# itxtx/normalizing-flows-study

Measured on AMD Instinct MI355X. Metric: log_prob samples/sec/GPU + test-NLL match; RealNVP d=2 and MAF d=63, higher is better.
Workload: dtype fp32

## Files before the change

### include/nfx.h

```cpp
#ifndef NFX_H
#define NFX_H

#include <stddef.h>
#include <stdint.h>

#ifdef __cplusplus
extern "C" {
#endif

#define NFX_ABI_VERSION 3

#define NFX_OK 0
#define NFX_EINVAL (-1)
#define NFX_EUNSUPPORTED (-2)
#define NFX_ELAUNCH (-3)

#define NFX_FORWARD 1
#define NFX_INVERSE (-1)

#define NFX_MAF_INVERSE 0
#define NFX_IAF_FORWARD 1
#define NFX_MAF_FORWARD 2
#define NFX_IAF_INVERSE 3

typedef struct NfxMlpRaw {
    const float* w[4];
    const float* b[4];
    const float* mask[4];
    const float* bn_w[3];
    const float* bn_b[3];
    const float* bn_rm[3];
    const float* bn_rv[3];
    float bn_eps;
    int n_layers;
} NfxMlpRaw;

int nfx_abi_version(void);
const char* nfx_last_error(void);
const char* nfx_last_kernel(void);
int nfx_debug_fill_lds(uint32_t bits, void* stream);

size_t nfx_affine_packed_floats(int d, int H);
int nfx_affine_pack(const NfxMlpRaw* s_net, const NfxMlpRaw* b_net, const float* mask, int d,
                    int H, float* packed, void* stream);
int nfx_affine_coupling(const float* packed, const float* in, float* out, float* log_det,
                        int64_t B, int d, int H, int direction, int accumulate, void* stream);
int nfx_affine_coupling_logprob(const float* packed, const float* in, float* out, float* log_det,
                                float* logp, double* sums, void* workspace, int64_t B, int d,
                                int H, int accumulate, void* stream);
#define NFX_AFFINE_AUTO 0
#define NFX_AFFINE_STREAMING 1
#define NFX_AFFINE_SMALL 2
int nfx_affine_kernel_policy(int policy);

int nfx_affine_chain_supported(int64_t B, int d, int H);
int nfx_affine_chain(const float* const* packs, int n_layers, const float* in, float* out,
                     float* log_det, int64_t B, int d, int H, int direction, int accumulate,
                     void* stream);
int nfx_affine_chain_logprob(const float* const* packs, int n_layers, const float* in, float* out,
                             float* log_det, float* logp, double* sums, void* workspace, int64_t B,
                             int d, int H, int accumulate, void* stream);
int nfx_affine_chain_sample(const float* const* packs, int n_layers, uint64_t seed, uint64_t* rng_state,
                            float* z, float* x, float* log_det, int64_t B, int d, int H, void* stream);

size_t nfx_spline_packed_floats(int d, int H, int K);
int nfx_spline_pack(const NfxMlpRaw* param_net, const float* mask, int d, int H, int K,
                    float* packed, void* stream);
int nfx_spline_coupling(const float* packed, const float* in, float* out, float* log_det,
                        int64_t B, int d, int H, int K, float bound, float min_bin_width,
                        float min_bin_height, float min_derivative, int rescale,
                        float data_min, float data_max, int direction, int accumulate,
                        void* stream);
int nfx_spline_coupling_logprob(const float* packed, const float* in, float* out, float* log_det,
                                float* logp, double* sums, void* workspace, int64_t B, int d,
                                int H, int K, float bound, float min_bin_width,
                                float min_bin_height, float min_derivative, int rescale,
                                float data_min, float data_max, int accumulate, void* stream);

int nfx_spline_chain_supported(int64_t B, int d, int H, int K);
int nfx_spline_chain(const float* const* packs, int n_layers, const float* in, float* out, float* log_det,
                     int64_t B, int d, int H, int K, float bound, float min_bin_width, float min_bin_height,
                     float min_derivative, int direction, int accumulate, void* stream);
int nfx_spline_chain_logprob(const float* const* packs, int n_layers, const float* in, float* out,
                             float* log_det, float* logp, double* sums, void* workspace, int64_t B, int d,
                             int H, int K, float bound, float min_bin_width, float min_bin_height,
                             float min_derivative, int accumulate, void* stream);
int nfx_spline_chain_sample(const float* const* packs, int n_layers, uint64_t seed, uint64_t* rng_state,
                            float* z, float* x, float* log_det, int64_t B, int d, int H, int K, float bound,
                            float min_bin_width, float min_bin_height, float min_derivative, void* stream);

int nfx_rqs_unit(const float* in, const float* widths, const float* heights,
                 const float* derivatives, float* out, float* log_det, int64_t N, int K,
                 float min_bin_width, float min_bin_height, float min_derivative, int inverse,
                 void* stream);
int nfx_rqs_unit_backward(const float* in, const float* widths, const float* heights,
                          const float* derivatives, const float* grad_out, const float* grad_log_det,
                          float* grad_in, float* grad_widths, float* grad_heights, float* grad_derivatives,
                          int64_t N, int K, float min_bin_width, float min_bin_height, float min_derivative,
                          int inverse, void* stream);

size_t nfx_arqs_packed_floats(int d, int H, int K);
int nfx_arqs_pack(const NfxMlpRaw* made, int d, int H, int K, float* packed, void* stream);
int nfx_arqs(const float* packed, const float* in, float* out, float* log_det, int64_t B, int d,
             int H, int K, float min_bin_width, float min_bin_height, float min_derivative,
             int rescale, double data_min, double data_max, int direction, int accumulate,
             void* stream);

int nfx_base_normal(uint64_t seed, uint64_t* rng_state, float* z, int64_t B, int d, void* stream);

size_t nfx_made_packed_floats(int d, int H);
int nfx_made_pack(const NfxMlpRaw* net, int d, int H, float* packed, void* stream);
int nfx_made_pack_parallel(const NfxMlpRaw* net, int d, int H, float* packed, void* stream);
int nfx_made_pack_sequential(int d, int H, float* packed, void* stream);
int nfx_made_affine(const float* packed, const float* in, float* out, float* log_det,
                    int64_t B, int d, int H, int variant, int accumulate, void* stream);
#define NFX_MADE_SEQ_AUTO 0
#define NFX_MADE_SEQ_SEGMENT 1
#define NFX_MADE_SEQ_WAVE 2
#define NFX_MADE_SEQ_PUSH 3
int nfx_made_seq_policy(int policy);
int nfx_made_affine_logprob(const float* packed, const float* in, float* out, float* log_det,
                            float* logp, double* sums, void* workspace, int64_t B, int d, int H,
                            int variant, int accumulate, void* stream);
int nfx_made_sample_supported(int d, int H, int variant);
int nfx_made_affine_sample(const float* packed, uint64_t seed, uint64_t* rng_state, float* z, float* x,
                           float* log_det, int64_t B, int d, int H, void* stream);

int nfx_made_pack_backward(const NfxMlpRaw* net, int d, int H, float* packed, void* stream);
size_t nfx_made_backward_factor_floats(int64_t B, int d, int H);
int64_t nfx_made_backward_max_batch(int d, int H);
int nfx_made_affine_backward(const float* packed, const float* in, const float* grad_out,
                             const float* grad_log_det, float* grad_in, float* factors, int64_t B,
                             int d, int H, int variant, void* stream);

int nfx_made_seq_backward(const float* packed, const float* in, const float* grad_out,
                          const float* grad_log_det, float* grad_in, float* factors, int64_t B,
                          int d, int H, int variant, void* stream);
int64_t nfx_made_factor_pitch(int64_t B);
size_t nfx_made_param_floats(int d, int H);
size_t nfx_made_wgrad_workspace_bytes(int64_t B, int d, int H);
int nfx_made_backward_weights(const float* factors, int64_t B, int d, int H,
                              const float* const* masks, float* grads, void* workspace,
                              void* stream);

size_t nfx_spline_backward_packed_floats(int d, int H, int K);
size_t nfx_spline_backward_param_floats(int d, int H, int K);
size_t nfx_spline_backward_workspace_bytes(int64_t B, int d, int H, int K);
int nfx_spline_pack_backward(const NfxMlpRaw* net, const float* mask, int d, int H, int K,
                             float* packed, void* stream);
int nfx_spline_coupling_backward(const float* packed, const float* mask, const float* in,
                                 const float* grad_out, const float* grad_log_det, float* grad_in,
                                 float* grads, void* workspace, int64_t B, int d, int H, int K,
                                 int n_transformed, float bound, float min_bin_width,
                                 float min_bin_height, float min_derivative, int direction,
                                 void* stream);

size_t nfx_affine_train_pack_floats(int d, int H);
size_t nfx_affine_train_stats_doubles(int H);
size_t nfx_affine_train_grad_doubles(int d, int H);
size_t nfx_affine_train_param_floats(int d, int H);
size_t nfx_affine_train_workspace_bytes(int64_t B, int d, int H);
int nfx_affine_train_pack(const NfxMlpRaw* s_net, const NfxMlpRaw* b_net, const float* mask,
                          const double* stats1, const double* stats2, int d, int H, float* tpack,
                          float* epack, void* stream);
int nfx_affine_train_stats(const float* tpack, const float* in, int64_t B, int d, int H, int layer,
                           double* stats, void* workspace, void* stream);
int nfx_affine_train_update_running(const double* stats1, const double* stats2,
                                    float* const* running_mean, float* const* running_var, int H,
                                    double momentum, void* stream);
int nfx_affine_train_update_running_counted(const double* stats1, const double* stats2,
                                            float* const* running_mean, float* const* running_var,
                                            int64_t* const* num_batches_tracked, int H,
                                            double momentum, void* stream);
int nfx_affine_train_backward(const float* tpack, const float* in, const float* grad_out,
                              const float* grad_log_det, float* grad_in, int64_t B, int d, int H,
                              int direction, int stage, const double* stats2, double* G,
                              void* workspace, void* stream);
int nfx_affine_train_assemble(const double* G, const double* stats1, const double* stats2, int d,
                              int H, float eps, float* grads, void* stream);
size_t nfx_affine_train_keep_floats(int64_t B, int d, int H);
int nfx_affine_train_stats_keep(const float* tpack, const float* in, int64_t B, int d, int H,
                                int layer, double* stats, void* workspace, float* keep,
                                void* stream);
int nfx_affine_train_backward_keep(const float* tpack, const float* in, const float* grad_out,
                                   const float* grad_log_det, float* grad_in, int64_t B, int d,
                                   int H, int direction, int stage, const double* stats2,
                                   double* G, void* workspace, const float* keep, void* stream);
int nfx_affine_train_output(const float* tpack, const float* in, const float* keep, float* out,
                            float* log_det, int64_t B, int d, int H, int direction, void* stream);
int nfx_affine_eval_stats(float* const* running_mean, float* const* running_var, int H,
                          double* stats1, double* stats2, void* stream);

size_t nfx_gauss_workspace_bytes(int64_t B);
int nfx_gauss_workspace_init(void* workspace, void* stream);
int nfx_gauss_logprob(const float* z, const float* log_det, float* logp, double* sums,
                      void* workspace, int64_t B, int d, void* stream);
int nfx_gauss_logprob_backward(const float* z, const float* grad_logp, float* grad_z, float* grad_log_det,
                               int64_t B, int d, void* stream);

size_t nfx_flowbn_workspace_bytes(int64_t B, int d);
int nfx_flowbn_apply(const float* in, float* out, float* log_det, const float* gamma, const float* beta,
                     const float* running_mean, const float* running_var, float eps, int64_t B, int d,
                     int direction, void* stream);
int nfx_flowbn_moments(const float* x, int64_t B, int d, double* stats, void* workspace, void* stream);
int nfx_flowbn_update_running(const double* stats, float* running_mean, float* running_var,
                              double momentum, int d, void* stream);
int nfx_flowbn_backward(const float* in, const float* grad_out, const float* grad_log_det, float* grad_in,
                        const float* gamma, const float* beta, const float* running_mean,
                        const float* running_var, float eps, float* grad_gamma, float* grad_beta,
                        int64_t B, int d, int direction, void* workspace, void* stream);


int nfx_linear_forward(const float* x, const float* w, const float* wmask, const float* b, const float* in_scale,
                       const float* post_scale, const float* post_shift, float* y, int64_t M, int K, int N,
                       int relu, void* stream);
int nfx_linear_backward_data(const float* gy, const float* w, const float* wmask, const float* act,
                             const float* out_scale, float* gx, int64_t M, int N, int K, int accumulate, void* stream);
size_t nfx_linear_workspace_bytes(int64_t M, int N, int K);
int nfx_linear_backward_weight(const float* gy, const float* x, const float* in_scale, const float* wmask, float* gw,
                               float* gb, int64_t M, int N, int K, void* workspace, void* stream);
int nfx_made_elem_forward(const float* x, const float* params, float* y, float* log_det, int64_t B, int d,
                          int variant, int accumulate, void* stream);
int nfx_made_elem_step(const float* x, const float* params, float* work, float* work_ld, int64_t B, int d, int i,
                       int variant, void* stream);
int nfx_made_elem_finish(const float* x, const float* work, const float* work_ld, float* y, float* log_det,
                         int64_t B, int d, int variant, int accumulate, void* stream);
int nfx_made_elem_backward(const float* x, const float* params, const float* gy, const float* gld, float* gparams,
                           float* gx, int64_t B, int d, int variant, void* stream);
int nfx_made_elem_seq_backward(const float* x, const float* params, const float* work, const float* lam,
                               const float* gy, const float* gld, float* out, int64_t B, int d, int variant, int mode,
                               void* stream);
int nfx_made_elem_seq_step_backward(const float* x, const float* params, const float* work, const float* work_ld,
                                    const float* lam, const float* grad_out, const float* grad_log_det,
                                    float* grad_params, float* grad_in, int64_t B, int d, int i, int variant,
                                    void* stream);
int nfx_made_elem_prefix(const float* work, float* out, int64_t B, int d, int i, void* stream);
int nfx_affine_elem_forward(const float* x, const float* s_raw, const float* b_raw, const float* mask, float* y,
                            float* log_det, int64_t B, int d, int direction, int accumulate, void* stream);
int nfx_affine_elem_backward(const float* x, const float* s_raw, const float* b_raw, const float* mask,
                             const float* gy, const float* gld, float* gs, float* gb, float* gx, int64_t B, int d,
                             int direction, void* stream);
int nfx_bn_prepare(const double* stats, const float* gamma, const float* beta, float* running_mean,
                   float* running_var, double eps, double momentum, int update_running, int N, float* mean,
                   float* invstd, float* scale, float* shift, void* stream);
int nfx_bn_apply_relu(const float* z, const float* scale, const float* shift, float* h, int64_t M, int N,
                      void* stream);
size_t nfx_bn_workspace_bytes(int64_t M, int N);
int nfx_bn_backward_sums(const float* g, const float* z, const float* mean, const float* invstd, double* sums,
                         int64_t M, int N, void* workspace, void* stream);
int nfx_bn_backward_apply(const float* g, const float* z, const float* mean, const float* invstd,
                          const float* gamma, const double* sums, const double* count, int train, float* gz,
                          int64_t M, int N, void* stream);
int nfx_arqs_step(const float* xr, const float* params, float* state, float* log_det, const float* gld, float* lam,
                  float* gparams, float* gx, int64_t B, int d, int K, int i, int direction, int mode,
                  float min_bin_width, float min_bin_height, float min_derivative, void* stream);
int nfx_arqs_bounds(const float* in, const float* bounds, float* out, int64_t B, int d, int mode, void* stream);
int nfx_spline_elem_forward(const float* x, const float* params, const float* mask, float* y, float* log_det,
                            int64_t B, int d, int K, float bound, float min_bin_width, float min_bin_height,
                            float min_derivative, int direction, int accumulate, void* stream);
int nfx_spline_elem_backward(const float* x, const float* params, const float* mask, const float* gy,
                             const float* gld, float* gparams, float* gx, int64_t B, int d, int K, float bound,
                             float min_bin_width, float min_bin_height, float min_derivative, int direction,
                             void* stream);
int nfx_spline_elem_forward_bounded(const float* x, const float* params, const float* mask, const float* bounds,
                                    float* y, float* log_det, int64_t B, int d, int K, float bound,
                                    float min_bin_width, float min_bin_height, float min_derivative, int direction,
                                    int accumulate, void* stream);
int nfx_spline_elem_backward_bounded(const float* x, const float* params, const float* mask, const float* bounds,
                                     const float* gy, const float* gld, float* gparams, float* gx, int64_t B, int d,
                                     int K, float bound, float min_bin_width, float min_bin_height,
                                     float min_derivative, int direction, void* stream);
int nfx_spline_rescale(const float* x, const float* bounds, float* xr, int64_t B, int d, float bound, void* stream);

size_t nfx_cnf_packed_floats(int d, int H);
int nfx_cnf_pack(const float* w1, const float* b1, const float* w2, const float* b2, const float* w3,
                 const float* b3, int d, int H, float* packed, void* stream);
int nfx_cnf_supported(int64_t B, int d, int H);
int nfx_cnf_integrate(const float* packed, const float* in, float* out, float* log_det, int64_t B, int d,
                      int H, float t_begin, float t_end, float step_size, int accumulate, void* stream);

int nfx_cnf_backward_supported(int64_t B, int d, int H);
size_t nfx_cnf_backward_packed_floats(int d, int H);
size_t nfx_cnf_trajectory_floats(int64_t B, int d, float t_begin, float t_end, float step_size);
size_t nfx_cnf_backward_workspace_floats(int64_t B, int d, int H);
size_t nfx_cnf_backward_slots(int64_t B, int d, int H);
size_t nfx_cnf_backward_block_threads(int64_t B, int d, int H);
int nfx_cnf_pack_backward(const float* w1, const float* b1, const float* w2, const float* b2, const float* w3,
                          const float* b3, int d, int H, float* packed, void* stream);
int nfx_cnf_integrate_save(const float* packed, const float* in, float* out, float* log_det, float* traj,
                           int64_t B, int d, int H, float t_begin, float t_end, float step_size, int accumulate,
                           void* stream);
int nfx_cnf_backward(const float* packed, const float* w1, const float* w2, const float* w3, const float* in,
                     const float* traj, const float* gy, const float* gld, float* gx, float* gw1, float* gb1,
                     float* gw2, float* gb2, float* gw3, float* gb3, float* workspace, int64_t B, int d, int H,
                     float t_begin, float t_end, float step_size, void* stream);

#define NFX_RESIDUAL_RELU 0
#define NFX_RESIDUAL_ELU 1
#define NFX_RESIDUAL_LEAKY_RELU 2
#define NFX_RESIDUAL_TANH 3
size_t nfx_residual_packed_floats(int d, int H);
int nfx_residual_supported(int64_t B, int d, int H, int activation);
int nfx_residual_pack(const float* w1, const float* b1, const float* u1, const float* v1, float c1, const float* w2,
                      const float* b2, const float* u2, const float* v2, float c2, const float* w3, const float* b3,
                      const float* u3, const float* v3, float c3, int d, int H, float* packed, void* stream);
int nfx_residual_flow(const float* packed, const float* in, float* out, float* log_det, int64_t B, int d, int H,
                      int activation, int direction, int neumann_terms, int max_iter, float tol, int accumulate,
                      void* stream);

int nfx_residual_backward_supported(int64_t B, int d, int H, int activation);
size_t nfx_residual_backward_packed_floats(int d, int H);
size_t nfx_residual_backward_workspace_floats(int64_t B, int d, int H);
size_t nfx_residual_backward_slots(int64_t B, int d, int H);
size_t nfx_residual_backward_block_threads(int64_t B, int d, int H);
int nfx_residual_pack_backward(const float* w1, const float* b1, const float* u1, const float* v1, float c1,
                               const float* w2, const float* b2, const float* u2, const float* v2, float c2,
                               const float* w3, const float* b3, const float* u3, const float* v3, float c3, int d,
                               int H, float* packed, void* stream);
int nfx_residual_backward(const float* packed, const float* z, const float* gy, const float* gld, float* gx,
                          float* gw1, float* gb1, float* gw2, float* gb2, float* gw3, float* gb3, float* workspace,
                          int64_t B, int d, int H, int activation, int direction, int neumann_terms, void* stream);

#define NFX_NAF_RELU 0
#define NFX_NAF_ELU 1
#define NFX_NAF_LEAKY_RELU 2
#define NFX_NAF_GELU 3
#define NFX_NAF_LAYER_NORM 1
#define NFX_NAF_RESIDUAL(l) (2 << (l))
typedef struct NfxNafLayer {
    const float* weight;
    const float* bias;
    const float* mask;
    const float* ln_weight;
    const float* ln_bias;
    float ln_eps;
    int residual;
} NfxNafLayer;
size_t nfx_naf_packed_floats(int d, int n_hidden, const int* widths);
int nfx_naf_supported(int64_t B, int d, int n_hidden, const int* widths, int activation, int flags);
int nfx_naf_pack(const NfxNafLayer* layers, int d, int n_hidden, const int* widths, float* packed, void* stream);
int nfx_naf_flow(const float* packed, const float* in, float* out, float* log_det, int64_t B, int d, int n_hidden,
                 const int* widths, int activation, int flags, float clamp_alpha, float clamp_log_scale,
                 int direction, int accumulate, void* stream);

size_t nfx_naf_wide_packed_floats(int d, int n_hidden, const int* widths);
int nfx_naf_wide_supported(int64_t B, int d, int n_hidden, const int* widths, int activation, int flags);
int nfx_naf_wide_pack(const NfxNafLayer* layers, int d, int n_hidden, const int* widths, float* packed,
                      void* stream);
int nfx_naf_wide_flow(const float* packed, const float* in, float* out, float* log_det, int64_t B, int d,
                      int n_hidden, const int* widths, int activation, int flags, float clamp_alpha,
                      float clamp_log_scale, int direction, int accumulate, void* stream);

typedef struct NfxNafLayerGrad {
    float* weight;
    float* bias;
    float* ln_weight;
    float* ln_bias;
} NfxNafLayerGrad;
int nfx_naf_backward_supported(int64_t B, int d, int n_hidden, const int* widths, int activation, int flags);
size_t nfx_naf_backward_packed_floats(int d, int n_hidden, const int* widths);
int nfx_naf_pack_backward(const NfxNafLayer* layers, int d, int n_hidden, const int* widths, float* packed,
                          void* stream);
size_t nfx_naf_backward_slots(int64_t B, int d, int n_hidden, const int* widths);
size_t nfx_naf_backward_block_threads(int64_t B, int d, int n_hidden, const int* widths);
size_t nfx_naf_backward_workspace_floats(int64_t B, int d, int n_hidden, const int* widths);
int nfx_naf_backward(const float* packed, const NfxNafLayer* layers, const float* x, const float* gz,
                     const float* gld, float* gx, const NfxNafLayerGrad* grads, float* workspace, int64_t B, int d,
                     int n_hidden, const int* widths, int activation, int flags, float clamp_alpha,
                     float clamp_log_scale, void* stream);

int nfx_lowrank_supported(int64_t B, int dim, int n_layers);
size_t nfx_lowrank_record_floats(int dim);
int nfx_lowrank_pack_planar(const float* w, const float* u_hat, const float* b, int dim, int max_iter, float tol,
                            float* record, void* stream);
int nfx_lowrank_pack_radial(const float* z0, const float* alpha_hat, const float* beta_hat, int dim, int max_iter,
                            float tol, float* record, void* stream);
int nfx_lowrank_pack_sylvester(const float* v, const float* R, const float* b, int dim, int num_householder,
                               int num_transforms, int max_iter, float tol, float* record, void* stream);
int nfx_lowrank_stack(const float* image, int n_layers, const float* x, float* out, float* log_det, int64_t B,
                      int dim, int direction, int accumulate, void* stream);

int nfx_lrbwd_supported(int64_t B, int dim, int n_layers, int direction);
size_t nfx_lrbwd_max_layers(int dim);
size_t nfx_lrbwd_chunk_rows(int dim);
size_t nfx_lrbwd_slots(int64_t B, int dim, int n_layers);
size_t nfx_lrbwd_workspace_floats(int64_t B, int dim, int n_layers);
int nfx_lrbwd_stack(const float* image, int n_layers, const float* point, const float* gv, const float* gld, float* gx,
                    float* workspace, int64_t B, int dim, int direction, void* stream);
int nfx_lrbwd_param_grads(const float* workspace, int64_t B, int dim, int n_layers, int layer, int kind,
                          const float* p0, const float* p1, const float* p2, float* g0, float* g1, float* g2,
                          int num_householder, int num_transforms, void* stream);

#ifdef __cplusplus
}
#endif

#endif
```

### normalizing-flows-study_amd/csrc/nfx_affine_kernel.h

```cpp
#pragma once
#include <type_traits>
#include <utility>

#include "nfx_common.h"

namespace nfx {

__host__ __device__ constexpr int up4(int v) { return (v + 3) & ~3; }

struct AffineLayout {
    int d, HT, KS1;
    int w1, b1, w2, b2, w3, b3, net, mask, total;
    int s;
};

constexpr uint32_t kAffineLiveElide = 0x100u;
struct AffineSplit {
    int w1, b1, b2, w3, b3, w2s, net, mask, ok, total;
};

__host__ __device__ constexpr AffineSplit affine_split(int d, int HT) {
    AffineSplit S{};
    int o = 0;
    S.w1 = o; o += HT * ((d + 1) / 2) * 64;
    S.b1 = o; o += HT * 32;
    S.b2 = o; o += HT * 32;
    S.w3 = o; o += d * HT * 32;
    S.b3 = o; o += up4(d);
    S.w2s = o; o += HT * 2 * HT * 768;
    S.net = o;
    S.mask = 2 * o;
    S.ok = S.mask + up4(d);
    S.total = S.ok + 4;
    return S;
}

__host__ __device__ constexpr bool affine_has_split(int d, int HT) { return d <= 8 && HT <= 2; }

__host__ __device__ constexpr AffineLayout affine_layout(int d, int HT) {
    AffineLayout L{};
    L.d = d;
    L.HT = HT;
    L.KS1 = (d + 1) / 2;
    int o = 0;
    L.w1 = o; o += HT * L.KS1 * 64;
    L.b1 = o; o += HT * 32;
    L.w2 = o; o += HT * HT * 16 * 64;
    L.b2 = o; o += HT * 32;
    if (d <= 8) {
        L.w3 = o; o += d * HT * 32;
        L.b3 = o; o += up4(d);
    } else {
        const int NJ = (d + 31) / 32;
        L.w3 = o; o += NJ * HT * 1024;
        L.b3 = o; o += NJ * 32;
    }
    L.net = o;
    L.mask = 2 * o;
    L.total = 2 * o + up4(d);
    L.s = L.total;
    if (affine_has_split(d, HT)) L.total += affine_split(d, HT).total;
    return L;
}

template <int D>
__device__ __forceinline__ void load_row(const float* __restrict__ p, float (&v)[D]) {
    if constexpr (D == 2) {
        float2 t = *reinterpret_cast<const float2*>(p);
        v[0] = t.x; v[1] = t.y;
    } else if constexpr (D == 4) {
        float4 t = *reinterpret_cast<const float4*>(p);
        v[0] = t.x; v[1] = t.y; v[2] = t.z; v[3] = t.w;
    } else {
#pragma unroll
        for (int j = 0; j < D; ++j) v[j] = p[j];
    }
}

template <int D>
__device__ __forceinline__ void store_row(float* __restrict__ p, const float (&v)[D]) {
    if constexpr (D == 2) {
        *reinterpret_cast<float2*>(p) = make_float2(v[0], v[1]);
    } else if constexpr (D == 4) {
        *reinterpret_cast<float4*>(p) = make_float4(v[0], v[1], v[2], v[3]);
    } else {
#pragma unroll
        for (int j = 0; j < D; ++j) p[j] = v[j];
    }
}

template <int HT, int D, int TILES = 2>
__device__ __forceinline__ void affine_net(const float* __restrict__ P, const AffineLayout& L,
                                           const float (&xb)[2][(D + 1) / 2], float (&res)[D]) {
    constexpr int KS1 = (D + 1) / 2;
    const int lane = lane_id(), h = lane >> 5;

    f32x16 h1[HT][2];
#pragma unroll
    for (int ht = 0; ht < HT; ++ht) {
        f32x16 a0, a1;
        load_bias16_x2(P + L.b1 + ht * 32, h, a0, a1);
#pragma unroll
        for (int ks = 0; ks < KS1; ++ks) {
            const float w = P[L.w1 + (ht * KS1 + ks) * 64 + lane];
            a0 = mfma32(w, xb[0][ks], a0);
            if constexpr (TILES == 2) a1 = mfma32(w, xb[1][ks], a1);
        }
#pragma unroll
        for (int r = 0; r < 16; ++r) {
            a0[r] = trelu(a0[r]);
            if constexpr (TILES == 2) a1[r] = trelu(a1[r]);
        }
        h1[ht][0] = a0;
        h1[ht][1] = a1;
    }

    float part[D][2];
#pragma unroll
    for (int j = 0; j < D; ++j) part[j][0] = part[j][1] = 0.f;
    const f32x4* wg = reinterpret_cast<const f32x4*>(P + L.w2) + lane;
#pragma unroll
    for (int hto = 0; hto < HT; ++hto) {
        f32x16 a0, a1;
        load_bias16_x2(P + L.b2 + hto * 32, h, a0, a1);
#pragma unroll
        for (int kt = 0; kt < HT; ++kt) {
#pragma unroll
            for (int rq = 0; rq < 4; ++rq) {
                const f32x4 w = wg[a_quad(a_tile(hto, kt, HT), rq) * 64];
#pragma unroll
                for (int rr = 0; rr < 4; ++rr) {
                    a0 = mfma32(w[rr], h1[kt][0][4 * rq + rr], a0);
                    if constexpr (TILES == 2) a1 = mfma32(w[rr], h1[kt][1][4 * rq + rr], a1);
                }
            }
        }
#pragma unroll
        for (int j = 0; j < D; ++j) {
            const f32x16 w3 = load_bias16(P + L.w3 + (j * HT + hto) * 32, h);
#pragma unroll
            for (int r = 0; r < 16; ++r) {
                part[j][0] = fmaf(w3[r], trelu(a0[r]), part[j][0]);
                if constexpr (TILES == 2) part[j][1] = fmaf(w3[r], trelu(a1[r]), part[j][1]);
            }
        }
    }
#pragma unroll
    for (int j = 0; j < D; ++j)
        res[j] = tclamp(halves_sum(part[j][0], part[j][1]) + P[L.b3 + j], -10.f, 10.f);
}

#ifndef NFX_SPLIT_TERMS
#define NFX_SPLIT_TERMS 6
#endif
typedef __bf16 bf16x8 __attribute__((ext_vector_type(8)));
typedef uint32_t u32x4 __attribute__((ext_vector_type(4)));

__device__ __forceinline__ f32x16 mfma_bf16(u32x4 a, u32x4 b, f32x16 c) {
    return __builtin_amdgcn_mfma_f32_32x32x16_bf16(__builtin_bit_cast(bf16x8, a), __builtin_bit_cast(bf16x8, b), c,
                                                    0, 0, 0);
}

__device__ __forceinline__ void split3(float x, uint32_t& u0, uint32_t& u1, uint32_t& u2) {
    u0 = __float_as_uint(x) & 0xffff0000u;
    const float r1 = x - __uint_as_float(u0);
    u1 = __float_as_uint(r1) & 0xffff0000u;
    u2 = __float_as_uint(r1 - __uint_as_float(u1));
}

__device__ __forceinline__ uint32_t pack_bf16(uint32_t lo, uint32_t hi) {
    return __builtin_amdgcn_perm(hi, lo, 0x07060302u);
}

__device__ __forceinline__ void split_block(const f32x16& a, int half, u32x4 (&xp)[3]) {
#pragma unroll
    for (int q = 0; q < 4; ++q) {
        uint32_t l0, l1, l2, h0, h1, h2;
        split3(a[8 * half + 2 * q], l0, l1, l2);
        split3(a[8 * half + 2 * q + 1], h0, h1, h2);
        xp[0][q] = pack_bf16(l0, h0);
        xp[1][q] = pack_bf16(l1, h1);
        xp[2][q] = pack_bf16(l2, h2);
    }
}

template <class F, int... I>
__device__ __forceinline__ void static_for_seq(F&& f, std::integer_sequence<int, I...>) {
    (f(std::integral_constant<int, I>{}), ...);
}
template <int N, class F>
__device__ __forceinline__ void static_for(F&& f) {
    static_for_seq(f, std::make_integer_sequence<int, N>{});
}

#if NFX_SPLIT_TERMS == 8
constexpr int kSplitTermW[8] = {2, 1, 2, 1, 0, 1, 0, 0}, kSplitTermX[8] = {1, 2, 0, 1, 2, 0, 1, 0};
#else
constexpr int kSplitTermW[6] = {2, 1, 0, 1, 0, 0}, kSplitTermX[6] = {0, 1, 2, 0, 1, 0};
#endif

template <int HT, int D, int TILES, bool LIVE>
__device__ __forceinline__ void affine_nets_split_pipe(const float* __restrict__ S, const AffineSplit& SL,
                                                       const float (&xb)[2][(D + 1) / 2], float (&sv)[D],
                                                       float (&bv)[D], uint32_t live_idx) {
    constexpr int KS1 = (D + 1) / 2;
    constexpr int NJ = LIVE ? (D + 1) / 2 : D;
    constexpr int NS = 2 * TILES;
    constexpr int KB = 2 * HT;
    constexpr int NT = NFX_SPLIT_TERMS;
    constexpr int NM = NT * HT;
    constexpr int NG = KB * NM;
    constexpr int NFI = 16 * HT;
    constexpr int NQ = 3 * HT;
    constexpr int WG0 = (NM - NQ) / 2;
    constexpr int L1G = (KB - 2) * NM;
    constexpr int L1P = L1G >= 2 ? L1G - 2 : 0;
    constexpr int HB0 = NM / 2;
    const int lane = lane_id(), h = lane >> 5;

    const float* Sn[NS];
    const u32x4* w2n[NS];
    f32x16 h1[NS][HT];
    uint32_t u[NS * KB][3][8];
    u32x4 xp[NS * KB][3];
    u32x4 w[NS * KB][HT][3];
    f32x16 hi[NS][HT], lo[NS][HT];
    f32x4 w3q[NS][HT][NJ][4];
    float r1[NS * KB][8], tf[NS][NFI];
    float part[2][NJ][2];
    int w3row[NJ];
#pragma unroll
    for (int j = 0; j < NJ; ++j) w3row[j] = (LIVE ? (int)((live_idx >> (4 * j)) & 7u) : j) * HT * 32;
#pragma unroll
    for (int n = 0; n < 2; ++n)
#pragma unroll
        for (int j = 0; j < NJ; ++j) part[n][j][0] = part[n][j][1] = 0.f;

    auto base = [&](int s) __attribute__((always_inline)) {
        Sn[s] = S + (s / TILES) * SL.net + opaque_zero();
        w2n[s] = reinterpret_cast<const u32x4*>(Sn[s] + SL.w2s) + lane;
    };
    auto l1_bias = [&](int s) __attribute__((always_inline)) {
#pragma unroll
        for (int ht = 0; ht < HT; ++ht) h1[s][ht] = load_bias16(Sn[s] + SL.b1 + ht * 32, h);
    };
    auto l1_mfma = [&](int s) __attribute__((always_inline)) {
#pragma unroll
        for (int ht = 0; ht < HT; ++ht)
#pragma unroll
            for (int ks = 0; ks < KS1; ++ks)
                h1[s][ht] = mfma32(Sn[s][SL.w1 + (ht * KS1 + ks) * 64 + lane], xb[s % TILES][ks], h1[s][ht]);
    };
    auto split_slot = [&](int b, int i) __attribute__((always_inline)) {
        const int s = b / KB, kb = b % KB, q = i / 3;
#pragma unroll
        for (int e = 2 * q; e < 2 * q + 2; ++e) {
            if (i % 3 == 0) {
                const float x = trelu(h1[s][kb >> 1][8 * (kb & 1) + e]);
                u[b][0][e] = __float_as_uint(x) & 0xffff0000u;
                r1[b][e] = x - __uint_as_float(u[b][0][e]);
            } else if (i % 3 == 1) {
                u[b][1][e] = __float_as_uint(r1[b][e]) & 0xffff0000u;
                u[b][2][e] = __float_as_uint(r1[b][e] - __uint_as_float(u[b][1][e]));
            }
        }
        if (i % 3 == 2) {
#pragma unroll
            for (int p = 0; p < 3; ++p) xp[b][p][q] = pack_bf16(u[b][p][2 * q], u[b][p][2 * q + 1]);
        }
    };
    auto w2_quad = [&](int b, int i) __attribute__((always_inline)) {
        const int s = b / KB, kb = b % KB, p = 2 - i / HT, hto = i % HT;
        w[b][hto][p] = w2n[s][((hto * KB + kb) * 3 + p) * 64];
    };
    auto w3_quads = [&](int s, int hto, int rq) __attribute__((always_inline)) {
#pragma unroll
        for (int j = 0; j < NJ; ++j)
            w3q[s][hto][j][rq] = *reinterpret_cast<const f32x4*>(Sn[s] + SL.w3 + w3row[j] + hto * 32 + 16 * h + 4 * rq);
    };
    auto fold_relu = [&](int s, int f) __attribute__((always_inline)) {
        tf[s][f] = trelu(hi[s][f / 16][f % 16] + lo[s][f / 16][f % 16]);
    };
    auto fold_fma = [&](int s, int f) __attribute__((always_inline)) {
        const int hto = f / 16, r = f % 16;
#pragma unroll
        for (int j = 0; j < NJ; ++j)
            part[s / TILES][j][s % TILES] = fmaf(w3q[s][hto][j][r / 4][r % 4], tf[s][f], part[s / TILES][j][s % TILES]);
    };
    constexpr auto fold_gap = [](int f) { return (((f | 1) + 1) * NG + NFI - 1) / NFI - 1; };
    constexpr auto w3_gap = [](int f) {
        const int g = (((f | 1) + 1) * NG + NFI - 1) / NFI - 1;
        return g >= 2 ? g - 2 : 0;
    };
    static_assert(fold_gap(NFI - 1) < NG && fold_gap(0) >= 1 && w3_gap(0) < fold_gap(0), "fold schedule");
    static_assert(WG0 >= 0 && WG0 + NQ <= NM && HB0 + HT <= NM - HT, "read schedule");
    static_assert(KB < 2 || L1G <= (KB - 1) * NM - 1, "layer 1 of the next stage precedes its first split");

    base(0);
    l1_bias(0);
#pragma unroll
    for (int i = 0; i < NQ; ++i) w2_quad(0, i);
    l1_mfma(0);
#pragma unroll
    for (int i = 0; i < 12; ++i) split_slot(0, i);

    static_for<NS>([&](auto sc) __attribute__((always_inline)) {
        constexpr int s = decltype(sc)::value;
        static_for<NG>([&](auto gc) __attribute__((always_inline)) {
            constexpr int g = decltype(gc)::value;
            constexpr int kb = g / NM, m = g % NM, b = s * KB + kb;
            constexpr int t = m / HT, hto = m % HT;
            __builtin_amdgcn_sched_barrier(0);
            if (t == NT - 1) {
                hi[s][hto] = mfma_bf16(w[b][hto][kSplitTermW[t]], xp[b][kSplitTermX[t]], hi[s][hto]);
            } else {
                lo[s][hto] = mfma_bf16(w[b][hto][kSplitTermW[t]], xp[b][kSplitTermX[t]],
                                       kb == 0 && t == 0 ? f32x16{} : lo[s][hto]);
            }
            __builtin_amdgcn_sched_barrier(0);
            if (g == 0 && s + 1 < NS) base(s + 1);
            if (b + 1 < NS * KB && m >= WG0 && m < WG0 + NQ) w2_quad(b + 1, m - WG0);
            if (kb == 0 && m >= HB0 && m < HB0 + HT)
                hi[s][m - HB0] = load_bias16(Sn[s] + SL.b2 + (m - HB0) * 32, h);
            if (s > 0) {
#pragma unroll
                for (int fq = 0; fq < NFI; fq += 4)
                    if (w3_gap(fq) == g) w3_quads(s - 1, fq / 16, (fq % 16) / 4);
            }
            if (s + 1 < NS && g == L1P) l1_bias(s + 1);
            if (s + 1 < NS && g == L1G) l1_mfma(s + 1);
            if (b + 1 < NS * KB) {
#pragma unroll
                for (int i = m * 12 / NM; i < (m + 1) * 12 / NM; ++i) split_slot(b + 1, i);
            }
            if (s > 0) {
#pragma unroll
                for (int f = 0; f < NFI; ++f)
                    if ((fold_gap(f) >= 1 ? fold_gap(f) - 1 : 0) == g) fold_relu(s - 1, f);
#pragma unroll
                for (int f = 0; f < NFI; ++f)
                    if (fold_gap(f) == g) fold_fma(s - 1, f);
            }
        });
    });
    __builtin_amdgcn_sched_barrier(0);
#pragma unroll
    for (int fq = 0; fq < NFI; fq += 4) w3_quads(NS - 1, fq / 16, (fq % 16) / 4);
#pragma unroll
    for (int f = 0; f < NFI; ++f) {
        fold_relu(NS - 1, f);
        fold_fma(NS - 1, f);
    }
    if constexpr (LIVE) {
#pragma unroll
        for (int j = 0; j < D; ++j) sv[j] = bv[j] = 0.f;
#pragma unroll
        for (int jj = 0; jj < NJ; ++jj) {
            const int o = (int)((live_idx >> (4 * jj)) & 15u);
            const float s = tclamp(halves_sum(part[0][jj][0], part[0][jj][1]) + Sn[0][SL.b3 + (o & 7)], -10.f, 10.f);
            const float b = tclamp(halves_sum(part[1][jj][0], part[1][jj][1]) + Sn[NS - 1][SL.b3 + (o & 7)], -10.f, 10.f);
#pragma unroll
            for (int j = 0; j < D; ++j) {
                sv[j] = o == j ? s : sv[j];
                bv[j] = o == j ? b : bv[j];
            }
        }
    } else {
#pragma unroll
        for (int j = 0; j < D; ++j) {
            sv[j] = tclamp(halves_sum(part[0][j][0], part[0][j][1]) + Sn[0][SL.b3 + j], -10.f, 10.f);
            bv[j] = tclamp(halves_sum(part[1][j][0], part[1][j][1]) + Sn[NS - 1][SL.b3 + j], -10.f, 10.f);
        }
    }
}

template <int KS1>
__device__ __forceinline__ bool affine_live_unit(const float (&xb)[2][KS1], const float (&mkb)[KS1]) {
    bool bad = false;
#pragma unroll
    for (int st = 0; st < 2; ++st)
#pragma unroll
        for (int ks = 0; ks < KS1; ++ks)
            bad = bad || (mkb[ks] == 1.f && (!(fabsf(xb[st][ks]) <= 1e33f) || __float_as_uint(xb[st][ks]) == 0x80000000u));
    return __builtin_amdgcn_ballot_w64(bad) == 0;
}

template <int HT, int D, int TILES = 2>
__device__ __forceinline__ void affine_net_split(const float* __restrict__ S, const AffineSplit& SL,
                                                 const float (&xb)[2][(D + 1) / 2], float (&res)[D]) {
    constexpr int KS1 = (D + 1) / 2;
    const int lane = lane_id(), h = lane >> 5;

    f32x16 h1[HT][2];
#pragma unroll
    for (int ht = 0; ht < HT; ++ht) {
        f32x16 a0, a1;
        load_bias16_x2(S + SL.b1 + ht * 32, h, a0, a1);
#pragma unroll
        for (int ks = 0; ks < KS1; ++ks) {
            const float w = S[SL.w1 + (ht * KS1 + ks) * 64 + lane];
            a0 = mfma32(w, xb[0][ks], a0);
            if constexpr (TILES == 2) a1 = mfma32(w, xb[1][ks], a1);
        }
#pragma unroll
        for (int r = 0; r < 16; ++r) {
            a0[r] = trelu(a0[r]);
            if constexpr (TILES == 2) a1[r] = trelu(a1[r]);
        }
        h1[ht][0] = a0;
        h1[ht][1] = a1;
    }

    float part[D][2];
#pragma unroll
    for (int j = 0; j < D; ++j) part[j][0] = part[j][1] = 0.f;
    auto fold = [&](int hto, const f32x16& a, int st) {
#pragma unroll
        for (int j = 0; j < D; ++j) {
            const f32x16 w3 = load_bias16(S + SL.w3 + (j * HT + hto) * 32, h);
#pragma unroll
            for (int r = 0; r < 16; ++r) part[j][st] = fmaf(w3[r], trelu(a[r]), part[j][st]);
        }
    };
    const u32x4* w2s = reinterpret_cast<const u32x4*>(S + SL.w2s) + lane;
#pragma unroll
    for (int st = 0; st < TILES; ++st) {
        u32x4 xp[2 * HT][3];
#pragma unroll
        for (int kb = 0; kb < 2 * HT; ++kb) split_block(h1[kb >> 1][st], kb & 1, xp[kb]);
        const u32x4* w2 = w2s + opaque_zero();
#pragma unroll
        for (int hto = 0; hto < HT; ++hto) {
            f32x16 hi = load_bias16(S + SL.b2 + hto * 32 + opaque_zero(), h), lo = {};
#pragma unroll
            for (int kb = 0; kb < 2 * HT; ++kb) {
                const int g = (hto * 2 * HT + kb) * 3;
                const u32x4 w[3] = {w2[g * 64], w2[(g + 1) * 64], w2[(g + 2) * 64]};
#if NFX_SPLIT_TERMS == 8
                lo = mfma_bf16(w[2], xp[kb][1], lo);
                lo = mfma_bf16(w[1], xp[kb][2], lo);
#endif
                lo = mfma_bf16(w[2], xp[kb][0], lo);
                lo = mfma_bf16(w[1], xp[kb][1], lo);
                lo = mfma_bf16(w[0], xp[kb][2], lo);
                lo = mfma_bf16(w[1], xp[kb][0], lo);
                lo = mfma_bf16(w[0], xp[kb][1], lo);
                hi = mfma_bf16(w[0], xp[kb][0], hi);
            }
            fold(hto, hi + lo, st);
        }
    }
#pragma unroll
    for (int j = 0; j < D; ++j)
        res[j] = tclamp(halves_sum(part[j][0], part[j][1]) + S[SL.b3 + j], -10.f, 10.f);
}

__host__ __device__ constexpr bool affine_split_piped(int HT, int D) { return HT == 2 && D <= 4; }

template <int HT, int D, int TILES, bool PIPE>
__device__ __forceinline__ void affine_nets_split(const float* __restrict__ S, const AffineSplit& SL,
                                                  const float* __restrict__ Pg, const AffineLayout& L,
                                                  const float (&xb)[2][(D + 1) / 2], float (&sv)[D], float (&bv)[D],
                                                  bool live = false, uint32_t live_idx = 0) {
    constexpr int KS1 = (D + 1) / 2;
    const bool wok = S[SL.ok] != 0.f;
    const float xs = S[SL.ok + 1];
    bool fast[2];
#pragma unroll
    for (int st = 0; st < 2; ++st) {
        bool bad = false;
#pragma unroll
        for (int ks = 0; ks < KS1; ++ks) bad = bad || !(fabsf(xb[st][ks]) <= xs);
        fast[st] = wok && __builtin_amdgcn_ballot_w64(bad) == 0;
    }
    if constexpr (PIPE) {
        bool full = !live;
        if (live) {
            affine_nets_split_pipe<HT, D, TILES, true>(S, SL, xb, sv, bv, live_idx);
            bool zero = true;
#pragma unroll
            for (int j = 0; j < D; ++j) zero = zero && fabsf(sv[j]) < 1e-30f;
            full = __builtin_amdgcn_ballot_w64(zero) != 0;
        }
        if (full) affine_nets_split_pipe<HT, D, TILES, false>(S, SL, xb, sv, bv, 0u);
    } else {
        affine_net_split<HT, D, TILES>(S, SL, xb, sv);
        __builtin_amdgcn_sched_barrier(0);
        affine_net_split<HT, D, TILES>(S + SL.net, SL, xb, bv);
    }
    if (!(fast[0] && (TILES == 1 || fast[1]))) {
        __builtin_amdgcn_sched_barrier(0);
        const float* P = Pg + opaque_zero();
        float s2[D], b2[D];
        affine_net<HT, D, TILES>(P, L, xb, s2);
        __builtin_amdgcn_sched_barrier(0);
        affine_net<HT, D, TILES>(P + L.net, L, xb, b2);
        if (!fast[lane_id() >> 5]) {
#pragma unroll
            for (int j = 0; j < D; ++j) {
                sv[j] = s2[j];
                bv[j] = b2[j];
            }
        }
    }
}

template <int HT, int D, int DIR, bool LOGP>
__global__ __launch_bounds__(256) void affine_coupling_kernel(
    const float* __restrict__ packed, const float* __restrict__ in, float* __restrict__ out,
    float* __restrict__ logdet, int64_t B, int accumulate, int64_t nchunks,
    float* __restrict__ logp, double* __restrict__ partials, double* __restrict__ sums, float cgauss) {
    constexpr AffineLayout L = affine_layout(D, HT);
    constexpr int KS1 = L.KS1;
    constexpr bool SPLIT = affine_has_split(D, HT);
    constexpr AffineSplit SL = affine_split(D, HT);
    constexpr int MASK = SPLIT ? SL.mask : L.mask;
    extern __shared__ f32x4 lds4[];
    {
        const f32x4* src = reinterpret_cast<const f32x4*>(packed + (SPLIT ? L.s : 0));
        for (int i = threadIdx.x; i < (SPLIT ? SL.total : L.total) / 4; i += 256) lds4[i] = src[i];
    }
    __syncthreads();
    const float* sm = reinterpret_cast<const float*>(lds4);

    const int lane = lane_id(), h = lane >> 5, col = lane & 31;
    const int64_t nwaves = (int64_t)gridDim.x * 4;
    float mk[D], mkb[KS1];
#pragma unroll
    for (int j = 0; j < D; ++j) mk[j] = sm[MASK + j];
#pragma unroll
    for (int ks = 0; ks < KS1; ++ks) mkb[ks] = (2 * ks + h < D) ? sm[MASK + 2 * ks + h] : 0.f;
    const int64_t wv = (int64_t)blockIdx.x * 4 + (threadIdx.x >> 6);
    const int64_t F = nchunks / nwaves, R = nchunks - F * nwaves;
    const bool split = 2 * R <= nwaves;
    const int64_t nfull = split ? F : F + (wv < R ? 1 : 0);
    const bool half = split && wv < 2 * R;
    const int64_t half_base = F * nwaves * 64 + wv * 32;

    struct Fetch {
        float xb[2][KS1];
        float xr[D];
        float ldin;
    };
    auto fetch = [&](int64_t u, Fetch& f) {
        const int64_t base = u < nfull ? (wv + u * nwaves) * 64 : half_base;
        const int nsamp = u < nfull ? 64 : (u == nfull && half ? 32 : 0);
#pragma unroll
        for (int st = 0; st < 2; ++st) {
            const int64_t s = base + 32 * st + col;
#pragma unroll
            for (int ks = 0; ks < KS1; ++ks) {
                const int k = 2 * ks + h;
                f.xb[st][ks] = (32 * st + col < nsamp && k < D && s < B) ? in[s * D + k] : 0.f;
            }
        }
        const int64_t so = base + lane;
        if (lane < nsamp && so < B) {
            load_row<D>(in + so * D, f.xr);
            f.ldin = accumulate ? logdet[so] : 0.f;
        } else {
#pragma unroll
            for (int j = 0; j < D; ++j) f.xr[j] = 0.f;
            f.ldin = 0.f;
        }
    };

    double lpacc = 0.0;
    auto unit = [&](auto tiles_c, int64_t base, const Fetch& cur) {
        constexpr int TILES = decltype(tiles_c)::value;
        const float* smi = sm + opaque_zero();
        float xb[2][KS1];
#pragma unroll
        for (int st = 0; st < 2; ++st) {
#pragma unroll
            for (int ks = 0; ks < KS1; ++ks) xb[st][ks] = cur.xb[st][ks] * mkb[ks];
        }

        float sv[D], bv[D];
        if constexpr (SPLIT) {
            affine_nets_split<HT, D, TILES, false>(smi, SL, packed, L, xb, sv, bv);
        } else {
            affine_net<HT, D, TILES>(smi, L, xb, sv);
            affine_net<HT, D, TILES>(smi + L.net, L, xb, bv);
        }

        const int64_t so = base + lane;
        if (lane < 32 * TILES && so < B) {
#pragma clang fp contract(off)
            float y[D];
            float ld = 0.f;
#pragma unroll
            for (int j = 0; j < D; ++j) {
                const float m = mk[j], om = 1.f - m;
                const float xa = cur.xr[j] * m;
                float t;
                if constexpr (DIR < 0) {
                    t = (cur.xr[j] - bv[j]) * exp_fast(-sv[j]);
                    ld = ld + om * (-sv[j]);
                } else {
                    t = cur.xr[j] * exp_fast(sv[j]) + bv[j];
                    ld = ld + om * sv[j];
                }
                const float v = xa + om * t;
                y[j] = nonfinite(v) ? 0.f : v;
            }
            if (nonfinite(ld)) ld = 0.f;
            store_row<D>(out + so * D, y);
            const float ldt = accumulate ? cur.ldin + ld : ld;
            logdet[so] = ldt;
            if constexpr (LOGP) {
                float m = gauss_sq0(y[0]);
#pragma unroll
                for (int j = 1; j < D; ++j) m = gauss_sq(m, y[j]);
                const float lp = gauss_lp(m, cgauss, ldt);
                logp[so] = lp;
                lpacc += (double)lp;
            }
        }
    };

    Fetch cur;
    fetch(0, cur);
    for (int64_t u = 0; u < nfull; ++u) {
        Fetch nxt;
        fetch(u + 1, nxt);
        unit(std::integral_constant<int, 2>{}, (wv + u * nwaves) * 64, cur);
        cur = nxt;
    }
    if (half) unit(std::integral_constant<int, 1>{}, half_base, cur);
    if constexpr (LOGP) {
        logp_commit<256>(lpacc, partials, sums, B);
    }
}


constexpr int kWideWaves = 4;

template <int HT>
__device__ __forceinline__ void wide_net(const float* __restrict__ P, const AffineLayout& L, const float* xt, int S,
                                         const float* __restrict__ mask, int d, f32x16 (&res)[2]) {
    const int lane = lane_id(), h = lane >> 5, col = lane & 31;
    f32x16 h1[HT];
#pragma unroll
    for (int ht = 0; ht < HT; ++ht) h1[ht] = load_bias16(P + L.b1 + ht * 32, h);
    for (int ks = 0; ks < L.KS1; ++ks) {
        const int k = 2 * ks + h;
        const float xb = k < d ? xt[col * S + k] * mask[k] : 0.f;
#pragma unroll
        for (int ht = 0; ht < HT; ++ht) h1[ht] = mfma32(P[L.w1 + (ht * L.KS1 + ks) * 64 + lane], xb, h1[ht]);
    }
#pragma unroll
    for (int ht = 0; ht < HT; ++ht)
#pragma unroll
        for (int r = 0; r < 16; ++r) h1[ht][r] = trelu(h1[ht][r]);
    f32x16 h2[HT];
#pragma unroll
    for (int hto = 0; hto < HT; ++hto) {
        f32x16 a = load_bias16(P + L.b2 + hto * 32, h);
#pragma unroll
        for (int kt = 0; kt < HT; ++kt)
#pragma unroll
            for (int rq = 0; rq < 4; ++rq) {
                const f32x4 w = *reinterpret_cast<const f32x4*>(P + L.w2 + (a_quad(a_tile(hto, kt, HT), rq) * 64 + lane) * 4);
#pragma unroll
                for (int rr = 0; rr < 4; ++rr) a = mfma32(w[rr], h1[kt][4 * rq + rr], a);
            }
#pragma unroll
        for (int r = 0; r < 16; ++r) a[r] = trelu(a[r]);
        h2[hto] = a;
    }
    const int NJ = (d + 31) / 32;
#pragma unroll
    for (int j = 0; j < 2; ++j) {
        if (j < NJ) {
            f32x16 a = load_bias16(P + L.b3 + j * 32, h);
#pragma unroll
            for (int kt = 0; kt < HT; ++kt)
#pragma unroll
                for (int rq = 0; rq < 4; ++rq) {
                    const f32x4 w = *reinterpret_cast<const f32x4*>(P + L.w3 + (a_quad(a_tile(j, kt, HT), rq) * 64 + lane) * 4);
#pragma unroll
                    for (int rr = 0; rr < 4; ++rr) a = mfma32(w[rr], h2[kt][4 * rq + rr], a);
                }
#pragma unroll
            for (int r = 0; r < 16; ++r) a[r] = tclamp(a[r], -10.f, 10.f);
            res[j] = a;
        } else {
            res[j] = f32x16{};
        }
    }
}

template <int HT, int DIR, bool LOGP>
__global__ __launch_bounds__(64 * kWideWaves) void affine_wide_kernel(
    const float* __restrict__ packed, const float* __restrict__ in, float* __restrict__ out,
    float* __restrict__ logdet, int64_t B, int d, int accumulate, int64_t ntiles,
    float* __restrict__ logp, double* __restrict__ partials, double* __restrict__ sums, float cgauss) {
    const AffineLayout L = affine_layout(d, HT);
    const int S = d | 1;
    extern __shared__ f32x4 lds4[];
    const int wave = __builtin_amdgcn_readfirstlane(threadIdx.x >> 6);
    float* xt = reinterpret_cast<float*>(lds4) + wave * 32 * S;
    const int lane = lane_id(), h = lane >> 5, col = lane & 31;
    const float* mask = packed + L.mask;
    double lpacc = 0.0;
    for (int64_t t = (int64_t)blockIdx.x * kWideWaves + wave; t < ntiles; t += (int64_t)gridDim.x * kWideWaves) {
        const int64_t base = t * 32;
        const int rows = (int)(B - base < 32 ? B - base : 32);
        const float* src = in + base * d;
        for (int i = lane; i < 32 * d; i += 64) {
            const int r = i / d, c = i - r * d;
            xt[r * S + c] = r < rows ? src[i] : 0.f;
        }
        const float ldin = (accumulate && lane < rows) ? logdet[base + lane] : 0.f;
        wave_lds_sync();
        const float* Pw = packed + opaque_zero();
        f32x16 sv[2], bv[2];
        wide_net<HT>(Pw, L, xt, S, mask, d, sv);
        wide_net<HT>(Pw + L.net, L, xt, S, mask, d, bv);
        float ldp = 0.f;
        {
#pragma clang fp contract(off)
#pragma unroll
            for (int j = 0; j < 2; ++j)
#pragma unroll
                for (int r = 0; r < 16; ++r) {
                    const int dim = 32 * j + crow(r, h);
                    if (dim < d) {
                        float* px = xt + col * S + dim;
                        const float xv = *px, m = mask[dim], om = 1.f - m;
                        float tv;
                        if constexpr (DIR < 0) {
                            tv = (xv - bv[j][r]) * exp_fast(-sv[j][r]);
                            ldp = ldp + om * (-sv[j][r]);
                        } else {
                            tv = xv * exp_fast(sv[j][r]) + bv[j][r];
                            ldp = ldp + om * sv[j][r];
                        }
                        const float v = xv * m + om * tv;
                        *px = nonfinite(v) ? 0.f : v;
                    }
                }
        }
        float ld = halves_sum(ldp, ldp);
        if (nonfinite(ld)) ld = 0.f;
        wave_lds_sync();
        float* dst = out + base * d;
        for (int i = lane; i < rows * d; i += 64) {
            const int r = i / d, c = i - r * d;
            dst[i] = xt[r * S + c];
        }
        if (lane < rows) {
            const float ldt = accumulate ? ldin + ld : ld;
            logdet[base + lane] = ldt;
            if constexpr (LOGP) {
                float m = gauss_sq0(xt[lane * S]);
                for (int c = 1; c < d; ++c) m = gauss_sq(m, xt[lane * S + c]);
                const float lp = gauss_lp(m, cgauss, ldt);
                logp[base + lane] = lp;
                lpacc += (double)lp;
            }
        }
        wave_lds_sync();
    }
    if constexpr (LOGP) {
        logp_commit<64 * kWideWaves>(lpacc, partials, sums, B);
    }
}

typedef void (*affine_kernel_t)(const float*, const float*, float*, float*, int64_t, int, int64_t,
                                float*, double*, double*, float);

template <int HT>
affine_kernel_t affine_pick_ht(int d, int dir, bool logp);

template <int HT>
affine_kernel_t affine_pick(int d, int dir, bool logp) {
    return pick_range<1, 8>(d, [=](auto D) -> affine_kernel_t {
        if (dir > 0) return affine_coupling_kernel<HT, D(), 1, false>;
        return logp ? affine_coupling_kernel<HT, D(), -1, true> : affine_coupling_kernel<HT, D(), -1, false>;
    });
}

int affine_split_pack(float* packed, int d, int H, hipStream_t s);

}
```

### normalizing-flows-study_amd/csrc/nfx_made.hip

```cpp
#include "nfx_made_kernel.h"
#include "nfx_made_wide_kernel.h"
#include <atomic>
#include <cstdlib>

#include "nfx_made_seqs_kernel.h"
#include "nfx_pack.h"

namespace nfx {

__global__ void made_pack_kernel(NfxMlpRaw net, int d, int H, float* packed) {
    const int HT = (H + 31) / 32;
    const MadeLayout L = made_layout(d, HT);
    const int Hp = L.Hp, G1 = 4 * L.NKC;
    for (int i = blockIdx.x * blockDim.x + threadIdx.x; i < L.total; i += gridDim.x * blockDim.x) {
        if (i >= L.s_deg) continue;
        float v = 0.f;
        if (i < L.b1) {
            int t = i - L.w1, rr = t & 3, lane = (t >> 2) & 63, g = (t >> 8) % G1, ht = (t >> 8) / G1;
            int row = 32 * ht + (lane & 31), col = 2 * (4 * g + rr) + (lane >> 5);
            v = (row < H && col < d) ? mlp_weight(net, 0, d, row, col) : 0.f;
        } else if (i < L.w2) {
            int row = acc_vec_row(i - L.b1);
            v = row < H ? mlp_bias(net, 0, row) : 0.f;
        } else if (i < L.b2 || (i >= L.w3 && i < L.b3)) {
            const int layer = i < L.b2 ? 1 : 2;
            const ATileElem e = a_tile_elem(i - (layer == 1 ? L.w2 : L.w3));
            int row = 32 * (e.tile / HT) + e.row, col = 32 * (e.tile % HT) + e.k;
            v = (row < H && col < H) ? mlp_weight(net, layer, H, row, col) : 0.f;
        } else if (i < L.w3 || (i >= L.b3 && i < L.w4)) {
            const int layer = i < L.w3 ? 1 : 2;
            int row = acc_vec_row(i - (layer == 1 ? L.b2 : L.b3));
            v = row < H ? mlp_bias(net, layer, row) : 0.f;
        } else if (i < L.b4) {
            const ATileElem e = a_tile_elem(i - L.w4);
            int jw = e.tile / HT, which = jw & 1, j = jw >> 1;
            int orow = 32 * j + e.row, col = 32 * (e.tile % HT) + e.k;
            v = (orow < d && col < H) ? mlp_weight(net, 3, H, which * d + orow, col) : 0.f;
        } else if (i < L.par_total) {
            int t = i - L.b4, jw = t >> 5, which = jw & 1, j = jw >> 1;
            int orow = 32 * j + acc_vec_row(t & 31);
            v = orow < d ? mlp_bias(net, 3, which * d + orow) : 0.f;
        } else if (i < L.s_b1) {
            int t = i - L.s_w1t, ii = t / Hp, a = t % Hp;
            v = (ii < d && a < H) ? mlp_weight(net, 0, d, a, ii) : 0.f;
        } else if (i < L.s_w2) {
            int a = i - L.s_b1;
            v = a < H ? mlp_bias(net, 0, a) : 0.f;
        } else if (i < L.s_b2 || (i >= L.s_w3 && i < L.s_b3)) {
            const int layer = i < L.s_b2 ? 1 : 2;
            int t = i - (layer == 1 ? L.s_w2 : L.s_w3), a = t / Hp, b = t % Hp;
            v = (a < H && b < H) ? mlp_weight(net, layer, H, a, b) : 0.f;
        } else if (i < L.s_w3 || (i >= L.s_b3 && i < L.s_w4)) {
            const int layer = i < L.s_w3 ? 1 : 2;
            int a = i - (layer == 1 ? L.s_b2 : L.s_b3);
            v = a < H ? mlp_bias(net, layer, a) : 0.f;
        } else if (i < L.s_b4) {
            int t = i - L.s_w4, row = t / Hp, a = t % Hp;
            v = (row < 2 * d && a < H) ? mlp_weight(net, 3, H, row, a) : 0.f;
        } else if (i < L.s_deg) {
            int row = i - L.s_b4;
            v = row < 2 * d ? mlp_bias(net, 3, row) : 0.f;
        }
        packed[i] = v;
    }
}

constexpr int kLiveThreads = 1024;

__global__ __launch_bounds__(kLiveThreads) void made_live_kernel(NfxMlpRaw net, int d, int H, float* packed) {
    const int HT = (H + 31) / 32;
    const MadeLayout L = made_layout(d, HT);
    {
        __shared__ int deg[256];
        const int Hp = L.Hp;
        for (int a0 = 0; a0 < Hp; a0 += kLiveThreads / 16) {
            const int a = a0 + (threadIdx.x >> 4), q = threadIdx.x & 15;
            int n = 0;
            if (a < H && net.mask[0]) {
                const float* row = net.mask[0] + (size_t)a * d;
#pragma unroll 4
                for (int j = q; j < d; j += 16) n += row[j] != 0.f ? 1 : 0;
            }
            n += __shfl_xor(n, 1);
            n += __shfl_xor(n, 2);
            n += __shfl_xor(n, 4);
            n += __shfl_xor(n, 8);
            if (q == 0 && a < Hp) deg[a] = a < H ? (net.mask[0] ? n - 1 : 0) : 1000000000;
        }
        __syncthreads();
        for (int a = threadIdx.x; a < Hp; a += kLiveThreads) {
            const int da = deg[a];
            int rank = 0;
            for (int b = 0; b < Hp; ++b) rank += (deg[b] < da || (deg[b] == da && b < a)) ? 1 : 0;
            packed[L.s_deg + a] = (float)da;
            packed[L.s_deg + Hp + rank] = (float)da;
            packed[L.s_deg + 2 * Hp + rank] = (float)a;
        }
    }
    int* nk = reinterpret_cast<int*>(packed);
    for (int i = threadIdx.x; i < 3 * HT + L.NJ; i += kLiveThreads) nk[L.nk1 + i] = 0;
    __shared__ double red[256];
    const int rows[4] = {H, H, H, 2 * d}, cols[4] = {d, H, H, H};
    const double tsafe = block_mlp_tsafe(net, 4, rows, cols, 1.0e37, red);
    if (threadIdx.x == 0) packed[L.tsafe] = (float)fmin(tsafe, 3.0e38);
}

__global__ __launch_bounds__(256) void made_extent_kernel(int d, int H, float* packed) {
    const int HT = (H + 31) / 32;
    const MadeLayout L = made_layout(d, HT);
    int* nk = reinterpret_cast<int*>(packed);
    const int n1 = HT * 4 * L.NKC, n23 = HT * HT * 4, n4 = L.NJ * 2 * HT * 4;
    const int lane = lane_id();
    for (int gi = blockIdx.x * 4 + (threadIdx.x >> 6); gi < n1 + 2 * n23 + n4; gi += gridDim.x * 4) {
        int off, word, ext;
        if (gi < n1) {
            const int ht = gi / (4 * L.NKC), g = gi % (4 * L.NKC);
            off = L.w1 + gi * 256;
            word = L.nk1 + ht;
            ext = g / 4 + 1;
        } else if (gi < n1 + 2 * n23) {
            const int t = (gi - n1) % n23, layer = (gi - n1) / n23;
            off = (layer == 0 ? L.w2 : L.w3) + t * 256;
            word = (layer == 0 ? L.nk2 : L.nk3) + t / (HT * 4);
            ext = (t % (HT * 4)) / 4 + 1;
        } else {
            const int t = gi - n1 - 2 * n23;
            off = L.w4 + t * 256;
            word = L.nk4 + t / (2 * HT * 4);
            ext = (t % (HT * 4)) / 4 + 1;
        }
        const f32x4 v = *reinterpret_cast<const f32x4*>(packed + off + 4 * lane);
        const bool nzl = v[0] != 0.f || v[1] != 0.f || v[2] != 0.f || v[3] != 0.f;
        if (__ballot(nzl) != 0 && lane == 0) atomicMax(&nk[word], ext);
    }
}

template <int HT>
made_seqs_kernel_t made_seqs_pick_ht(int variant, bool logp) {
    if (variant == NFX_MAF_FORWARD) return made_seqs_kernel<HT, NFX_MAF_FORWARD, false>;
    return logp ? made_seqs_kernel<HT, NFX_IAF_INVERSE, true> : made_seqs_kernel<HT, NFX_IAF_INVERSE, false>;
}
template made_seqs_kernel_t made_seqs_pick_ht<1>(int, bool);
template made_seqs_kernel_t made_seqs_pick_ht<2>(int, bool);

template <int HT, int VAR>
static made_seq_kernel_t seq_var() {
    return made_seq_kernel<HT, VAR>;
}

template <int HT>
made_seq_kernel_t made_seq_pick_ht(int variant) {
    return variant == NFX_MAF_FORWARD ? seq_var<HT, NFX_MAF_FORWARD>() : seq_var<HT, NFX_IAF_INVERSE>();
}
template made_seq_kernel_t made_seq_pick_ht<1>(int);
template made_seq_kernel_t made_seq_pick_ht<2>(int);
template made_seq_kernel_t made_seq_pick_ht<3>(int);
template made_seq_kernel_t made_seq_pick_ht<4>(int);

static made_par_kernel_t pick_par(int HT, bool wlds, int variant) {
    return pick_range<1, 4>(HT, [=](auto HT_) { return made_pick_ht<HT_()>(wlds, variant); });
}

static made_par_kernel_t pick_tile(int HT, bool wlds, int variant, bool logp) {
    return pick_range<1, 4>(HT, [=](auto HT_) { return made_tile_pick_ht<HT_()>(wlds, variant, logp); });
}

static made_seq_kernel_t pick_seq(int HT, int variant) {
    return pick_range<1, 4>(HT, [=](auto HT_) { return made_seq_pick_ht<HT_()>(variant); });
}

int made_big_launch(const float* packed, const float* in, float* out, float* log_det, int64_t B, int d, int H,
                    int variant, int accumulate, hipStream_t s);

constexpr size_t kLdsBytes = 160 * 1024;
constexpr int kTileMaxD = 64;

}

using namespace nfx;

extern "C" size_t nfx_made_packed_floats(int d, int H) {
    if (d <= 0 || H <= 0) return 0;
    return (size_t)made_layout(d, (H + 31) / 32).total;
}

namespace nfx {
int made_pack_seqp(int d, int H, float* packed, hipStream_t s);
static int made_pack_seq(int d, int H, float* packed, hipStream_t s) {
    const int HT = (H + 31) / 32;
    if (HT > 2) return NFX_OK;
    if (HT == 1) made_seqs_image_kernel<1><<<64, 256, 0, s>>>(packed, d, H);
    else made_seqs_image_kernel<2><<<64, 256, 0, s>>>(packed, d, H);
    int rc = check_launch("made_seqs_image_kernel");
    if (rc) return rc;
    if (HT == 1) made_seqs_chunk_kernel<1><<<1, 64, 0, s>>>(packed, d, H);
    else made_seqs_chunk_kernel<2><<<1, 64, 0, s>>>(packed, d, H);
    rc = check_launch("made_seqs_chunk_kernel");
    if (rc) return rc;
    return made_pack_seqp(d, H, packed, s);
}
}

extern "C" int nfx_made_pack_parallel(const NfxMlpRaw* net, int d, int H, float* packed, void* stream) {
    if (!net || !packed) return set_error(NFX_EINVAL, "made_pack: null pointer");
    if (d <= 0 || d > 4096 || H <= 0 || H > 256)
        return set_error(NFX_EUNSUPPORTED, "made_pack: d=%d H=%d outside d<=4096, H<=256", d, H);
    if (net->n_layers != 4) return set_error(NFX_EINVAL, "made_pack: MADE has 4 masked layers (got %d)", net->n_layers);
    for (int l = 0; l < 4; ++l)
        if (!net->w[l]) return set_error(NFX_EINVAL, "made_pack: layer %d weight is null", l);
    const int total = (int)nfx_made_packed_floats(d, H);
    int blocks = (total + 255) / 256;
    if (blocks > 2048) blocks = 2048;
    made_pack_kernel<<<blocks, 256, 0, (hipStream_t)stream>>>(*net, d, H, packed);
    int rc = check_launch("made_pack_kernel");
    if (rc) return rc;
    made_live_kernel<<<1, kLiveThreads, 0, (hipStream_t)stream>>>(*net, d, H, packed);
    rc = check_launch("made_live_kernel");
    if (rc) return rc;
    {
        const int HT = (H + 31) / 32;
        const MadeLayout L = made_layout(d, HT);
        const int groups = HT * 4 * L.NKC + 2 * HT * HT * 4 + L.NJ * 2 * HT * 4;
        made_extent_kernel<<<(groups + 3) / 4, 256, 0, (hipStream_t)stream>>>(d, H, packed);
    }
    return check_launch("made_extent_kernel");
}

extern "C" int nfx_made_pack_sequential(int d, int H, float* packed, void* stream) {
    if (!packed) return set_error(NFX_EINVAL, "made_pack_sequential: null pointer");
    if (d <= 0 || d > 4096 || H <= 0 || H > 256)
        return set_error(NFX_EUNSUPPORTED, "made_pack_sequential: d=%d H=%d outside d<=4096, H<=256", d, H);
    return made_pack_seq(d, H, packed, (hipStream_t)stream);
}

extern "C" int nfx_made_pack(const NfxMlpRaw* net, int d, int H, float* packed, void* stream) {
    const int rc = nfx_made_pack_parallel(net, d, H, packed, stream);
    if (rc) return rc;
    return made_pack_seq(d, H, packed, (hipStream_t)stream);
}

namespace nfx {
int made_seqw_launch(const float* packed, const float* in, float* out, float* log_det, int64_t B, int d, int H,
                     int variant, int accumulate, float* logp, double* partials, double* sums, bool fused,
                     int* grid_out, hipStream_t s);
int made_seqp_launch(const float* packed, const float* in, float* out, float* log_det, int64_t B, int d, int H,
                     int variant, int accumulate, float* logp, double* partials, double* sums, bool fused,
                     hipStream_t s);
}

static std::atomic<int>& made_seq_policy() {
    static std::atomic<int> v{[] {
        const char* e = getenv("NFX_MADE_SEQ_POLICY");
        return e ? atoi(e) : NFX_MADE_SEQ_AUTO;
    }()};
    return v;
}

namespace nfx {
int made_seq_policy_get() { return made_seq_policy().load(std::memory_order_relaxed); }
}

static bool tile_path(int d, int HT, int variant) {
    return (variant == NFX_MAF_INVERSE || variant == NFX_IAF_FORWARD) && d > 0 && d <= kTileMaxD && HT >= 1 && HT <= 4;
}

struct TileConfig {
    int nw;
    bool wlds;
    size_t lds;
};
static TileConfig tile_config(const MadeLayout& L, int64_t ntiles, bool fused) {
    int nw = 8;
    if (!fused && ntiles < 4 * (int64_t)num_cus()) nw = (int)((ntiles + num_cus() - 1) / num_cus());
    const size_t wbytes = (size_t)L.par_total * sizeof(float);
    const size_t tiles = nw * 32 * (size_t)kTileStride * sizeof(float);
    const bool wlds = nw == 8 && wbytes + tiles <= kLdsBytes;
    return {nw, wlds, (wlds ? wbytes : 0) + tiles};
}

static int made_launch(const float* packed, const float* in, float* out, float* log_det, int64_t B,
                       int d, int H, int variant, int accumulate, float* logp, double* sums,
                       void* workspace, hipStream_t s) {
    const bool fused = sums != nullptr;
    if (B < 0 || d <= 0 || H <= 0) return set_error(NFX_EINVAL, "made_affine: bad shape");
    if (d > 4096 || H > 256) return set_error(NFX_EUNSUPPORTED, "made_affine: d=%d H=%d outside d<=4096, H<=256", d, H);
    if (variant < NFX_MAF_INVERSE || variant > NFX_IAF_INVERSE)
        return set_error(NFX_EINVAL, "made_affine: unknown variant %d", variant);
    const int HT = (H + 31) / 32;
    if (HT > 4) {
        if (fused) return set_error(NFX_EUNSUPPORTED, "made_affine_logprob: no fused log_prob for H=%d > 128", H);
        if (B == 0) return NFX_OK;
        if (!packed || !in || !out || !log_det) return set_error(NFX_EINVAL, "made_affine: null pointer");
        if (in == out) return set_error(NFX_EINVAL, "made_affine: in and out must not alias");
        return made_big_launch(packed, in, out, log_det, B, d, H, variant, accumulate, s);
    }
    const MadeLayout L = made_layout(d, HT);
    const bool parallel = variant == NFX_MAF_INVERSE || variant == NFX_IAF_FORWARD;
    const size_t wide_lds_bytes = (size_t)wide_lds(L, HT).total * sizeof(float);
    const bool wide = parallel && d > kTileMaxD && HT <= 2 && wide_lds_bytes <= kLdsBytes;
    const bool seqs = (variant == NFX_MAF_FORWARD || variant == NFX_IAF_INVERSE) && HT <= 2;
    if (fused && !((variant == NFX_MAF_INVERSE && (d <= kTileMaxD || wide)) || (variant == NFX_IAF_INVERSE && seqs)))
        return set_error(NFX_EUNSUPPORTED,
                         "made_affine_logprob: fused log_prob needs MAF inverse with d <= %d or H <= 64, "
                         "or IAF inverse with H <= 64", kTileMaxD);
    if (fused && B > 0 && (!logp || !workspace)) return set_error(NFX_EINVAL, "made_affine_logprob: null logp/workspace");
    if (B == 0) return fused ? gauss_finish(reinterpret_cast<double*>(workspace), 0, sums, 0, s) : NFX_OK;
    if (!packed || !in || !out || !log_det) return set_error(NFX_EINVAL, "made_affine: null pointer");
    if (in == out) return set_error(NFX_EINVAL, "made_affine: in and out must not alias");
    double* partials = reinterpret_cast<double*>(workspace);
    if (wide) {
        const int64_t nchunks = (B + 63) / 64;
        const int nw = nchunks < (int64_t)kWideWaves * num_cus() ? 4 : kWideWaves;
        const size_t lds_nw = (size_t)wide_lds(L, HT, nw).total * sizeof(float);
        made_par_kernel_t k = HT == 1 ? made_wide_pick_ht<1>(variant, fused, nw) : made_wide_pick_ht<2>(variant, fused, nw);
        int rc = prepare_lds((const void*)k, lds_nw);
        if (rc) return rc;
        int grid = resident_grid((const void*)k, 64 * nw, lds_nw, (nchunks + nw - 1) / nw);
        if (grid > kMaxPartials) grid = kMaxPartials;
        k<<<grid, 64 * nw, lds_nw, s>>>(packed, in, out, log_det, B, d, accumulate, nchunks, logp, partials,
                                        sums, gauss_const(d));
        return check_launch("made_wide_kernel");
    }
    if (tile_path(d, HT, variant)) {
        const int64_t ntiles = (B + 31) / 32;
        const TileConfig c = tile_config(L, ntiles, fused);
        made_par_kernel_t k = pick_tile(HT, c.wlds, variant, fused);
        if (!k) return set_error(NFX_EUNSUPPORTED, "made_affine: no kernel for H=%d", H);
        int rc = prepare_lds((const void*)k, c.lds);
        if (rc) return rc;
        int grid = resident_grid((const void*)k, 64 * c.nw, c.lds, (ntiles + c.nw - 1) / c.nw);
        if (grid > kMaxPartials) grid = kMaxPartials;
        k<<<grid, 64 * c.nw, c.lds, s>>>(packed, in, out, log_det, B, d, accumulate, ntiles, logp, partials, sums,
                                         gauss_const(d));
        return check_launch("made_tile_kernel");
    }
    if (variant == NFX_MAF_INVERSE || variant == NFX_IAF_FORWARD) {
        const size_t wbytes = (size_t)L.par_total * sizeof(float);
        const size_t stage8 = 8 * (size_t)kStageFloats * sizeof(float);
        const bool wlds = wbytes + stage8 <= kLdsBytes;
        made_par_kernel_t k = pick_par(HT, wlds, variant);
        if (!k) return set_error(NFX_EUNSUPPORTED, "made_affine: no kernel for H=%d", H);
        const int threads = wlds ? 512 : 256;
        const size_t lds = wlds ? wbytes + stage8 : 4 * (size_t)kStageFloats * sizeof(float);
        int rc = prepare_lds((const void*)k, lds);
        if (rc) return rc;
        const int64_t nchunks = (B + 63) / 64;
        const int nw = threads / 64;
        const int grid = resident_grid((const void*)k, threads, lds, (nchunks + nw - 1) / nw);
        k<<<grid, threads, lds, s>>>(packed, in, out, log_det, B, d, accumulate, nchunks, nullptr, nullptr, nullptr,
                                     0.f);
        return check_launch("made_parallel_kernel");
    }
    const int seq_pol = made_seq_policy().load(std::memory_order_relaxed);
    const bool push_auto = seq_pol == NFX_MADE_SEQ_AUTO && d > 32 && B <= 4096 * (int64_t)num_cus() / 256;
    if (seqs && (seq_pol == NFX_MADE_SEQ_PUSH || push_auto) && L.ps > 0)
        return made_seqp_launch(packed, in, out, log_det, B, d, H, variant, accumulate, logp, partials, sums, fused, s);
    if (seqs && (seq_pol == NFX_MADE_SEQ_PUSH || seq_pol == NFX_MADE_SEQ_WAVE || (seq_pol == NFX_MADE_SEQ_AUTO && B <= 2048 * (int64_t)num_cus() / 256))) {
        int grid = 0;
        return made_seqw_launch(packed, in, out, log_det, B, d, H, variant, accumulate, logp, partials, sums, fused,
                                &grid, s);
    }
    if (seqs) {
        made_seqs_kernel_t k = HT == 1 ? made_seqs_pick_ht<1>(variant, fused) : made_seqs_pick_ht<2>(variant, fused);
        const size_t lds = (size_t)seqs_lds(L.Hp).total * sizeof(float);
        int rc = prepare_lds((const void*)k, lds);
        if (rc) return rc;
        const int threads = kSeqsThreads;
        int grid = resident_grid((const void*)k, threads, lds, (B + 4 * kSeqsWaves - 1) / (4 * kSeqsWaves));
        if (grid > kMaxPartials) grid = kMaxPartials;
        k<<<grid, threads, lds, s>>>(packed, in, out, log_det, B, d, H, accumulate, logp, partials, sums,
                                     gauss_const(d));
        return check_launch("made_seqs_kernel");
    }
    made_seq_kernel_t k = pick_seq(HT, variant);
    if (!k) return set_error(NFX_EUNSUPPORTED, "made_affine: no sequential kernel for H=%d", H);
    const size_t lds = 2 * 64 * (size_t)(L.Hp + 4) * sizeof(float);
    int rc = prepare_lds((const void*)k, lds);
    if (rc) return rc;
    const int64_t grid = (B + 63) / 64;
    k<<<(unsigned)grid, 64, lds, s>>>(packed, in, out, log_det, B, d, H, accumulate);
    return check_launch("made_seq_kernel");
}

extern "C" int nfx_made_seq_policy(int policy) {
    if (policy < 0) return made_seq_policy().load();
    if (policy > NFX_MADE_SEQ_PUSH) return set_error(NFX_EINVAL, "made_seq_policy: unknown policy %d", policy);
    return made_seq_policy().exchange(policy);
}

extern "C" int nfx_made_affine(const float* packed, const float* in, float* out, float* log_det,
                               int64_t B, int d, int H, int variant, int accumulate, void* stream) {
    return made_launch(packed, in, out, log_det, B, d, H, variant, accumulate, nullptr, nullptr, nullptr,
                       (hipStream_t)stream);
}

extern "C" int nfx_made_affine_logprob(const float* packed, const float* in, float* out, float* log_det,
                                       float* logp, double* sums, void* workspace, int64_t B, int d,
                                       int H, int variant, int accumulate, void* stream) {
    if (!sums) return set_error(NFX_EINVAL, "made_affine_logprob: null sums");
    return made_launch(packed, in, out, log_det, B, d, H, variant, accumulate, logp, sums, workspace,
                       (hipStream_t)stream);
}

extern "C" int nfx_made_sample_supported(int d, int H, int variant) {
    return (H > 0 && tile_path(d, (H + 31) / 32, variant) && variant == NFX_IAF_FORWARD) ? 1 : 0;
}

extern "C" int nfx_made_affine_sample(const float* packed, uint64_t seed, uint64_t* rng_state, float* z, float* x,
                                      float* log_det, int64_t B, int d, int H, void* stream) {
    if (B < 0 || d <= 0 || H <= 0) return set_error(NFX_EINVAL, "made_affine_sample: bad shape");
    if (!nfx_made_sample_supported(d, H, NFX_IAF_FORWARD))
        return set_error(NFX_EUNSUPPORTED, "made_affine_sample: d=%d H=%d outside the tile kernel (d <= %d, H <= 128)",
                         d, H, kTileMaxD);
    if (B == 0) return NFX_OK;
    if (!packed || !rng_state || !z || !x || !log_det) return set_error(NFX_EINVAL, "made_affine_sample: null pointer");
    if (z == x) return set_error(NFX_EINVAL, "made_affine_sample: z and x must not alias");
    const int HT = (H + 31) / 32;
    const MadeLayout L = made_layout(d, HT);
    const int64_t ntiles = (B + 31) / 32;
    const TileConfig c = tile_config(L, ntiles, false);
    made_sample_kernel_t k =
        pick_range<1, 4>(HT, [=](auto HT_) { return made_tile_sample_pick_ht<HT_()>(c.wlds); });
    int rc = prepare_lds((const void*)k, c.lds);
    if (rc) return rc;
    int grid = resident_grid((const void*)k, 64 * c.nw, c.lds, (ntiles + c.nw - 1) / c.nw);
    if (grid > kMaxPartials) grid = kMaxPartials;
    k<<<grid, 64 * c.nw, c.lds, (hipStream_t)stream>>>(packed, nullptr, x, log_det, B, d, 0, ntiles, nullptr, nullptr,
                                                       nullptr, 0.f, MadeDraw{seed, rng_state, z});
    return check_launch("made_tile_kernel");
}
```

### normalizing-flows-study_amd/csrc/nfx_made_kernel.h

```cpp
#pragma once
#include "nfx_common.h"
#include "nfx_rng.h"

namespace nfx {

struct MadeLayout {
    int d, HT, Hp, NKC, NJ;
    int w1, b1, w2, b2, w3, b3, w4, b4;
    int par_total;
    int s_w1t, s_b1, s_w2, s_b2, s_w3, s_b3, s_w4, s_b4, s_deg;
    int nk1, nk2, nk3, nk4, tsafe;
    int t4, t3, t2, t1;
    int rimg;
    int sw1, sw4, sb4;
    int ctab;
    int ps, pw4, pw1, pb4, pw23, ptb, ptab;
    int total;
};

__host__ __device__ constexpr int made_up4(int v) { return (v + 3) & ~3; }

__host__ __device__ constexpr int seqs_w4_stride(int Hp) { return 2 * Hp + 4; }
constexpr int kSeqsPadRows = 64;
__host__ __device__ constexpr int seqs_max_chunks(int d, int Hp) { return d / 8 + 2 * Hp + 8; }
constexpr int kSeqpMaxS = 16;
__host__ __device__ constexpr int seqp_slots(int d, int HT) {
    return (HT <= 2 && d <= 64 * kSeqpMaxS) ? (d + 63) / 64 : 0;
}
__host__ __device__ constexpr int seqp_max_chunks(int d, int Hp) { return (d + 63) / 64 + 3 * Hp + 4; }

__host__ __device__ constexpr MadeLayout made_layout(int d, int HT) {
    MadeLayout L{};
    L.d = d;
    L.HT = HT;
    L.Hp = 32 * HT;
    L.NKC = (d + 31) / 32;
    L.NJ = (d + 31) / 32;
    int o = 0;
    L.w1 = o; o += HT * 4 * L.NKC * 256;
    L.b1 = o; o += HT * 32;
    L.w2 = o; o += HT * HT * 1024;
    L.b2 = o; o += HT * 32;
    L.w3 = o; o += HT * HT * 1024;
    L.b3 = o; o += HT * 32;
    L.w4 = o; o += L.NJ * 2 * HT * 1024;
    L.b4 = o; o += L.NJ * 2 * 32;
    L.par_total = o;
    L.s_w1t = o; o += made_up4(d * L.Hp);
    L.s_b1 = o; o += L.Hp;
    L.s_w2 = o; o += L.Hp * L.Hp;
    L.s_b2 = o; o += L.Hp;
    L.s_w3 = o; o += L.Hp * L.Hp;
    L.s_b3 = o; o += L.Hp;
    L.s_w4 = o; o += made_up4(2 * d * L.Hp);
    L.s_b4 = o; o += made_up4(2 * d);
    L.s_deg = o; o += 3 * L.Hp;
    L.nk1 = o; o += HT;
    L.nk2 = o; o += HT;
    L.nk3 = o; o += HT;
    L.nk4 = o; o += L.NJ;
    L.tsafe = o; o += 1;
    o = made_up4(o);
    L.t4 = o; o += HT * 2 * L.NJ * 1024;
    L.t3 = o; o += HT * HT * 1024;
    L.t2 = o; o += HT * HT * 1024;
    L.t1 = o; o += L.NKC * HT * 1024;
    L.rimg = o; o += HT <= 2 ? 2 * L.Hp * L.Hp + 5 * L.Hp : 0;
    o = made_up4(o);
    const int rows = HT <= 2 ? d + kSeqsPadRows : 0;
    L.sw1 = o; o += made_up4(rows * L.Hp);
    L.sw4 = o; o += made_up4(rows * seqs_w4_stride(L.Hp));
    L.sb4 = o; o += made_up4(2 * rows);
    L.ctab = o; o += HT <= 2 ? 8 * seqs_max_chunks(d, L.Hp) : 0;
    const int PS = seqp_slots(d, HT);
    L.ps = PS;
    L.pw4 = o; o += L.Hp * ((PS + 1) / 2) * 256;
    L.pw1 = o; o += L.Hp * ((PS + 3) / 4) * 256;
    L.pb4 = o; o += PS * 128;
    L.pw23 = o; o += PS ? 2 * L.Hp * L.Hp : 0;
    L.ptb = o; o += PS ? 4 * L.Hp : 0;
    L.ptab = o; o += PS ? 16 * seqp_max_chunks(d, L.Hp) : 0;
    L.total = o;
    return L;
}

constexpr int kStageStride = 33;
constexpr int kTileStride = 65;
constexpr int kStageFloats = 64 * kStageStride;

template <int VAR>
__device__ __forceinline__ float made_affine(float xv, float mu, float al, float& acc) {
#pragma clang fp contract(off)
    if constexpr (VAR == NFX_MAF_INVERSE) {
        const float a = tclamp(al, -3.f, 3.f);
        acc = acc + a;
        const float z = (xv - mu) * exp_fast(-a);
        return nonfinite(z) ? 0.f : z;
    } else {
        const float a = tclamp(al, -2.f, 2.f);
        const float m = tclamp(mu, -10.f, 10.f);
        acc = acc + a;
        const float y = xv * exp_fast(a) + m;
        return nonfinite(y) ? xv : y;
    }
}

__device__ __forceinline__ void stage_in(const float* __restrict__ in, int64_t base, int d, int64_t B,
                                         int dim0, float* st) {
    const int lane = lane_id();
#pragma unroll 8
    for (int i = 0; i < 32; ++i) {
        const int idx = i * 64 + lane;
        const int s = idx >> 5, dd = idx & 31;
        const int64_t row = base + s;
        const int dim = dim0 + dd;
        st[s * kStageStride + dd] = (row < B && dim < d) ? in[row * d + dim] : 0.f;
    }
}

__device__ __forceinline__ void stage_out(float* __restrict__ out, int64_t base, int d, int64_t B,
                                          int dim0, const float* st) {
    const int lane = lane_id();
#pragma unroll 8
    for (int i = 0; i < 32; ++i) {
        const int idx = i * 64 + lane;
        const int s = idx >> 5, dd = idx & 31;
        const int64_t row = base + s;
        const int dim = dim0 + dd;
        if (row < B && dim < d) out[row * d + dim] = st[s * kStageStride + dd];
    }
}


template <int HT>
__device__ __forceinline__ void made_hidden(const float* __restrict__ W, int woff, int boff,
                                            const f32x16 (&hin)[HT][2], f32x16 (&hout)[HT][2]) {
    const int lane = lane_id(), h = lane >> 5;
#pragma unroll
    for (int hto = 0; hto < HT; ++hto) {
        f32x16 a0, a1;
        load_bias16_x2(W + boff + hto * 32, h, a0, a1);
#pragma unroll
        for (int kt = 0; kt < HT; ++kt) {
#pragma unroll
            for (int rq = 0; rq < 4; ++rq) {
                const f32x4 w = *reinterpret_cast<const f32x4*>(W + woff + (a_quad(a_tile(hto, kt, HT), rq) * 64 + lane) * 4);
#pragma unroll
                for (int rr = 0; rr < 4; ++rr) {
                    a0 = mfma32(w[rr], hin[kt][0][4 * rq + rr], a0);
                    a1 = mfma32(w[rr], hin[kt][1][4 * rq + rr], a1);
                }
            }
        }
#pragma unroll
        for (int r = 0; r < 16; ++r) {
            a0[r] = trelu(a0[r]);
            a1[r] = trelu(a1[r]);
        }
        hout[hto][0] = a0;
        hout[hto][1] = a1;
    }
}

template <int HT, bool WLDS, int VAR>
__global__ __launch_bounds__(WLDS ? 512 : 256) void made_parallel_kernel(
    const float* __restrict__ packed, const float* __restrict__ in, float* __restrict__ out,
    float* __restrict__ logdet, int64_t B, int d, int accumulate, int64_t nchunks,
    float* __restrict__ , double* __restrict__ , double* __restrict__ ,
    float ) {
    constexpr int NWAVE = WLDS ? 8 : 4;
    const MadeLayout L = made_layout(d, HT);
    extern __shared__ f32x4 lds4[];
    float* lds = reinterpret_cast<float*>(lds4);
    const int wave = threadIdx.x >> 6;
    float* stg;
    if constexpr (WLDS) {
        const f32x4* src = reinterpret_cast<const f32x4*>(packed);
        for (int i = threadIdx.x; i < L.par_total / 4; i += NWAVE * 64) lds4[i] = src[i];
        stg = lds + L.par_total + wave * kStageFloats;
        __syncthreads();
    } else {
        stg = lds + wave * kStageFloats;
    }
    const int lane = lane_id(), h = lane >> 5, col = lane & 31;
    const int64_t nwaves = (int64_t)gridDim.x * NWAVE;

    for (int64_t c = (int64_t)blockIdx.x * NWAVE + wave; c < nchunks; c += nwaves) {
        const int64_t base = c * 64;
        const float* W = (WLDS ? lds : packed) + opaque_zero();

        f32x16 h1[HT][2];
#pragma unroll
        for (int ht = 0; ht < HT; ++ht) load_bias16_x2(W + L.b1 + ht * 32, h, h1[ht][0], h1[ht][1]);
        for (int kc = 0; kc < L.NKC; ++kc) {
            stage_in(in, base, d, B, 32 * kc, stg);
            wave_lds_sync();
#pragma unroll
            for (int g = 0; g < 4; ++g) {
                f32x4 w[HT];
#pragma unroll
                for (int ht = 0; ht < HT; ++ht)
                    w[ht] = *reinterpret_cast<const f32x4*>(W + L.w1 + ((ht * 4 * L.NKC + kc * 4 + g) * 64 + lane) * 4);
#pragma unroll
                for (int rr = 0; rr < 4; ++rr) {
                    const int k = 8 * g + 2 * rr + h;
                    const float b0 = stg[col * kStageStride + k];
                    const float b1 = stg[(32 + col) * kStageStride + k];
#pragma unroll
                    for (int ht = 0; ht < HT; ++ht) {
                        h1[ht][0] = mfma32(w[ht][rr], b0, h1[ht][0]);
                        h1[ht][1] = mfma32(w[ht][rr], b1, h1[ht][1]);
                    }
                }
            }
            wave_lds_sync();
        }
#pragma unroll
        for (int ht = 0; ht < HT; ++ht) {
#pragma unroll
            for (int r = 0; r < 16; ++r) {
                h1[ht][0][r] = trelu(h1[ht][0][r]);
                h1[ht][1][r] = trelu(h1[ht][1][r]);
            }
        }
        f32x16 h2[HT][2];
        made_hidden<HT>(W, L.w2, L.b2, h1, h2);
        made_hidden<HT>(W, L.w3, L.b3, h2, h1);

        float acc0 = 0.f, acc1 = 0.f;
        for (int j = 0; j < L.NJ; ++j) {
            f32x16 mu0, mu1, al0, al1;
            load_bias16_x2(W + L.b4 + (j * 2 + 0) * 32, h, mu0, mu1);
            load_bias16_x2(W + L.b4 + (j * 2 + 1) * 32, h, al0, al1);
#pragma unroll
            for (int kt = 0; kt < HT; ++kt) {
#pragma unroll
                for (int rq = 0; rq < 4; ++rq) {
                    const f32x4 wm = *reinterpret_cast<const f32x4*>(
                        W + L.w4 + (a_quad(a_tile(j * 2 + 0, kt, HT), rq) * 64 + lane) * 4);
                    const f32x4 wa = *reinterpret_cast<const f32x4*>(
                        W + L.w4 + (a_quad(a_tile(j * 2 + 1, kt, HT), rq) * 64 + lane) * 4);
#pragma unroll
                    for (int rr = 0; rr < 4; ++rr) {
                        const float b0 = h1[kt][0][4 * rq + rr], b1 = h1[kt][1][4 * rq + rr];
                        mu0 = mfma32(wm[rr], b0, mu0);
                        mu1 = mfma32(wm[rr], b1, mu1);
                        al0 = mfma32(wa[rr], b0, al0);
                        al1 = mfma32(wa[rr], b1, al1);
                    }
                }
            }
            stage_in(in, base, d, B, 32 * j, stg);
            wave_lds_sync();
#pragma unroll
            for (int r = 0; r < 16; ++r) {
                const int row = crow(r, h);
                if (32 * j + row < d) {
                    float* p0 = stg + col * kStageStride + row;
                    float* p1 = stg + (32 + col) * kStageStride + row;
                    *p0 = made_affine<VAR>(*p0, mu0[r], al0[r], acc0);
                    *p1 = made_affine<VAR>(*p1, mu1[r], al1[r], acc1);
                }
            }
            wave_lds_sync();
            stage_out(out, base, d, B, 32 * j, stg);
            wave_lds_sync();
        }
        float s = halves_sum(acc0, acc1);
        const int64_t so = base + lane;
        if (so < B) {
            float ld;
            if constexpr (VAR == NFX_MAF_INVERSE) {
                ld = -s;
                if (nonfinite(ld)) ld = 0.f;
                ld = tclamp(ld, -100.f, 100.f);
            } else {
                ld = s;
                if (nonfinite(ld)) ld = 0.f;
                ld = tclamp(ld, -50.f, 50.f);
            }
            logdet[so] = accumulate ? logdet[so] + ld : ld;
        }
    }
}


template <int HT, int VAR>
__global__ __launch_bounds__(64) void made_seq_kernel(
    const float* __restrict__ packed, const float* __restrict__ in, float* __restrict__ out,
    float* __restrict__ logdet, int64_t B, int d, int H, int accumulate) {
    constexpr int Hp = 32 * HT;
    constexpr int RS = Hp + 4;
    const MadeLayout L = made_layout(d, HT);
    extern __shared__ f32x4 lds4[];
    float* h1s = reinterpret_cast<float*>(lds4);
    float* h2s = h1s + 64 * RS;
    const int lane = threadIdx.x;
    const int64_t s = (int64_t)blockIdx.x * 64 + lane;
    const bool valid = s < B;
    const float* P = packed;

    float pre1[Hp], h3[Hp];
#pragma unroll
    for (int a = 0; a < Hp; ++a) {
        pre1[a] = P[L.s_b1 + a];
        h3[a] = 0.f;
        h1s[lane * RS + a] = 0.f;
        h2s[lane * RS + a] = 0.f;
    }
    float ld = 0.f;
    bool poison = false;
    int p = 0;
    const float* ord = P + L.s_deg;

    for (int i = 0; i < d; ++i) {
        float mu = 0.f, al = 0.f;
        const float* w_mu = P + L.s_w4 + (size_t)i * Hp;
        const float* w_al = P + L.s_w4 + (size_t)(d + i) * Hp;
#pragma unroll
        for (int a = 0; a < Hp; ++a) {
            mu = fmaf(w_mu[a], h3[a], mu);
            al = fmaf(w_al[a], h3[a], al);
        }
        mu = mu + P[L.s_b4 + i];
        al = al + P[L.s_b4 + d + i];
        if (poison) { mu = __builtin_nanf(""); al = mu; }
        const float xin = valid ? in[s * d + i] : 0.f;
        float xi;
        if constexpr (VAR == NFX_MAF_FORWARD) {
            const float a = tclamp(al, -3.f, 3.f);
            xi = xin * exp_fast(a) + mu;
            ld = ld + a;
            if (valid) out[s * d + i] = nonfinite(xi) ? 0.f : xi;
        } else {
            const float a = tclamp(al, -2.f, 2.f);
            const float m = tclamp(mu, -10.f, 10.f);
            xi = (xin - m) * exp_fast(-a);
            ld = ld - a;
            if (valid) out[s * d + i] = nonfinite(xi) ? xin : xi;
        }
        if (nonfinite(xi)) poison = true;
        const float* w1c = P + L.s_w1t + (size_t)i * Hp;
#pragma unroll
        for (int a = 0; a < Hp; ++a) pre1[a] = fmaf(w1c[a], xi, pre1[a]);
        int q = p;
        while (q < H && (int)ord[Hp + q] == i) ++q;
        if (q > p) {
            for (int k = p; k < q; ++k) {
                const int a = (int)ord[2 * Hp + k];
                float v = 0.f;
#pragma unroll
                for (int b = 0; b < Hp; ++b) v = (b == a) ? pre1[b] : v;
                h1s[lane * RS + a] = trelu(v);
            }
            for (int k = p; k < q; ++k) {
                const int a = (int)ord[2 * Hp + k];
                const float* w = P + L.s_w2 + (size_t)a * Hp;
                float v = 0.f;
#pragma unroll
                for (int b = 0; b < Hp; b += 4) {
                    const f32x4 hv = *reinterpret_cast<const f32x4*>(h1s + lane * RS + b);
                    v = fmaf(w[b], hv[0], v);
                    v = fmaf(w[b + 1], hv[1], v);
                    v = fmaf(w[b + 2], hv[2], v);
                    v = fmaf(w[b + 3], hv[3], v);
                }
                h2s[lane * RS + a] = trelu(v + P[L.s_b2 + a]);
            }
            for (int k = p; k < q; ++k) {
                const int a = (int)ord[2 * Hp + k];
                const float* w = P + L.s_w3 + (size_t)a * Hp;
                float v = 0.f;
#pragma unroll
                for (int b = 0; b < Hp; b += 4) {
                    const f32x4 hv = *reinterpret_cast<const f32x4*>(h2s + lane * RS + b);
                    v = fmaf(w[b], hv[0], v);
                    v = fmaf(w[b + 1], hv[1], v);
                    v = fmaf(w[b + 2], hv[2], v);
                    v = fmaf(w[b + 3], hv[3], v);
                }
                v = trelu(v + P[L.s_b3 + a]);
#pragma unroll
                for (int b = 0; b < Hp; ++b) h3[b] = (b == a) ? v : h3[b];
            }
            p = q;
        }
    }
    if (valid) {
        if (nonfinite(ld)) ld = 0.f;
        ld = (VAR == NFX_MAF_FORWARD) ? tclamp(ld, -100.f, 100.f) : tclamp(ld, -50.f, 50.f);
        logdet[s] = accumulate ? logdet[s] + ld : ld;
    }
}

typedef void (*made_seq_kernel_t)(const float*, const float*, float*, float*, int64_t, int, int, int);


template <int HT>
__device__ __forceinline__ void made_hidden1(const float* __restrict__ W, int woff, int boff,
                                             const f32x16 (&hin)[HT], f32x16 (&hout)[HT]) {
    const int lane = lane_id(), h = lane >> 5;
    f32x16 a[HT];
#pragma unroll
    for (int hto = 0; hto < HT; ++hto) {
        a[hto] = load_bias16(W + boff + hto * 32, h);
    }
#pragma unroll
    for (int kt = 0; kt < HT; ++kt) {
#pragma unroll
        for (int rq = 0; rq < 4; ++rq) {
            f32x4 w[HT];
#pragma unroll
            for (int hto = 0; hto < HT; ++hto)
                w[hto] = *reinterpret_cast<const f32x4*>(W + woff + (a_quad(a_tile(hto, kt, HT), rq) * 64 + lane) * 4);
#pragma unroll
            for (int rr = 0; rr < 4; ++rr) {
#pragma unroll
                for (int hto = 0; hto < HT; ++hto) a[hto] = mfma32(w[hto][rr], hin[kt][4 * rq + rr], a[hto]);
            }
        }
    }
#pragma unroll
    for (int hto = 0; hto < HT; ++hto) {
#pragma unroll
        for (int r = 0; r < 16; ++r) a[hto][r] = trelu(a[hto][r]);
        hout[hto] = a[hto];
    }
}

template <int HT, int NK>
__device__ __forceinline__ f32x16 hidden_tile(const float* __restrict__ W, int woff, int boff, int hto,
                                              const f32x16 (&hin)[HT]) {
    const int lane = lane_id(), h = lane >> 5;
    f32x16 a = load_bias16(W + boff + hto * 32, h);
#pragma unroll
    for (int kt = 0; kt < NK; ++kt) {
#pragma unroll
        for (int rq = 0; rq < 4; ++rq) {
            const f32x4 w = *reinterpret_cast<const f32x4*>(W + woff + (a_quad(a_tile(hto, kt, HT), rq) * 64 + lane) * 4);
#pragma unroll
            for (int rr = 0; rr < 4; ++rr) a = mfma32(w[rr], hin[kt][4 * rq + rr], a);
        }
    }
#pragma unroll
    for (int r = 0; r < 16; ++r) a[r] = trelu(a[r]);
    return a;
}

template <int HT, int N>
__device__ __forceinline__ f32x16 hidden_tile_n(int n, const float* __restrict__ W, int woff, int boff,
                                                int hto, const f32x16 (&hin)[HT]) {
    if constexpr (N == 0) {
        return hidden_tile<HT, 0>(W, woff, boff, hto, hin);
    } else {
        if (n >= N) return hidden_tile<HT, N>(W, woff, boff, hto, hin);
        return hidden_tile_n<HT, N - 1>(n, W, woff, boff, hto, hin);
    }
}

template <int HT>
__device__ __forceinline__ void made_hidden_nk(const float* __restrict__ W, int woff, int boff,
                                               const f32x16 (&hin)[HT], f32x16 (&hout)[HT],
                                               const int (&nk)[HT], bool full) {
    if (full) {
        made_hidden1<HT>(W, woff, boff, hin, hout);
        return;
    }
#pragma unroll
    for (int hto = 0; hto < HT; ++hto) hout[hto] = hidden_tile_n<HT, HT>(nk[hto], W, woff, boff, hto, hin);
}

template <int HT, int NK>
__device__ __forceinline__ void out_pair(const float* __restrict__ W, const MadeLayout& L, int j,
                                         const f32x16 (&hin)[HT], f32x16& mu, f32x16& al) {
    const int lane = lane_id(), h = lane >> 5;
    mu = load_bias16(W + L.b4 + (j * 2 + 0) * 32, h);
    al = load_bias16(W + L.b4 + (j * 2 + 1) * 32, h);
#pragma unroll
    for (int kt = 0; kt < NK; ++kt) {
#pragma unroll
        for (int rq = 0; rq < 4; ++rq) {
            const f32x4 wm = *reinterpret_cast<const f32x4*>(
                W + L.w4 + (a_quad(a_tile(j * 2 + 0, kt, HT), rq) * 64 + lane) * 4);
            const f32x4 wa = *reinterpret_cast<const f32x4*>(
                W + L.w4 + (a_quad(a_tile(j * 2 + 1, kt, HT), rq) * 64 + lane) * 4);
#pragma unroll
            for (int rr = 0; rr < 4; ++rr) {
                mu = mfma32(wm[rr], hin[kt][4 * rq + rr], mu);
                al = mfma32(wa[rr], hin[kt][4 * rq + rr], al);
            }
        }
    }
}

template <int HT, int N>
__device__ __forceinline__ void out_pair_n(int n, const float* __restrict__ W, const MadeLayout& L, int j,
                                           const f32x16 (&hin)[HT], f32x16& mu, f32x16& al) {
    if constexpr (N == 0) {
        out_pair<HT, 0>(W, L, j, hin, mu, al);
    } else {
        if (n >= N) {
            out_pair<HT, N>(W, L, j, hin, mu, al);
            return;
        }
        out_pair_n<HT, N - 1>(n, W, L, j, hin, mu, al);
    }
}

struct MadeDraw {
    uint64_t seed;
    uint64_t* rng;
    float* z;
};
__device__ __forceinline__ const MadeDraw& made_draw_arg(const MadeDraw& a) { return a; }
__device__ __forceinline__ void made_draw_tile(float (&pf)[32], int64_t tt, int64_t ntiles, int64_t B, int d,
                                               uint64_t seed, uint64_t off) {
    const int lane = lane_id();
    const bool live = tt < ntiles;
#pragma unroll
    for (int r = 0; r < 32; ++r) {
        const int64_t row = tt * 32 + r;
        pf[r] = 0.f;
        if (live && row < B) {
            const float v = base_value(row, lane, seed, off);
            pf[r] = lane < d ? v : 0.f;
        }
    }
}

template <int HT, bool WLDS, int VAR, bool LOGP, bool SAMPLE = false, typename... DRAW>
__global__ __launch_bounds__(512) void made_tile_kernel(
    const float* __restrict__ packed, const float* __restrict__ in, float* __restrict__ out,
    float* __restrict__ logdet, int64_t B, int d, int accumulate, int64_t ntiles,
    float* __restrict__ logp, double* __restrict__ partials, double* __restrict__ sums, float cgauss,
    DRAW... draw) {
    static_assert(sizeof...(DRAW) == (SAMPLE ? 1 : 0), "SAMPLE kernels take one MadeDraw");
    static_assert(!SAMPLE || (VAR == NFX_IAF_FORWARD && !LOGP), "SAMPLE: the IAF forward pass");
    const MadeLayout L = made_layout(d, HT);
    constexpr int S = kTileStride;
    extern __shared__ f32x4 lds4[];
    float* lds = reinterpret_cast<float*>(lds4);
    const int wave = __builtin_amdgcn_readfirstlane(threadIdx.x >> 6);
    const int nwg = LOGP ? 8 : (int)(blockDim.x >> 6);
    if constexpr (WLDS) {
        const f32x4* src = reinterpret_cast<const f32x4*>(packed);
        for (int i = threadIdx.x; i < L.par_total / 4; i += 64 * nwg) lds4[i] = src[i];
    }
    float* xt = lds + (WLDS ? L.par_total : 0) + wave * 32 * S;
    if constexpr (WLDS) __syncthreads();
    const int lane = lane_id(), h = lane >> 5, col = lane & 31;
    const int64_t nwaves = (int64_t)gridDim.x * nwg;
    const int voff = lane < d ? lane * 4 : (1 << 30);
    const int rowb = d * 4;
    const int* nkp = reinterpret_cast<const int*>(packed);
    int nk1[HT], nk2[HT], nk3[HT];
    bool full2 = true, full3 = true;
#pragma unroll
    for (int i = 0; i < HT; ++i) {
        nk1[i] = nkp[L.nk1 + i];
        nk2[i] = nkp[L.nk2 + i];
        nk3[i] = nkp[L.nk3 + i];
        full2 = full2 && nk2[i] >= HT;
        full3 = full3 && nk3[i] >= HT;
    }
    const float tsafe = packed[L.tsafe];

    int64_t t = (int64_t)blockIdx.x * nwg + wave;
    double lpacc = 0.0;
    float pf[32];
    float ldpf = 0.f;
    uint64_t draw_off = 0;
    if constexpr (SAMPLE) {
        draw_off = rng_offset(made_draw_arg(draw...).rng);
        made_draw_tile(pf, t, ntiles, B, d, made_draw_arg(draw...).seed, draw_off);
    } else {
        if (accumulate && t < ntiles && lane < 32 && t * 32 + col < B) ldpf = logdet[t * 32 + col];
        const int64_t rows = t < ntiles ? (B - t * 32 < 32 ? B - t * 32 : 32) : 0;
        const auto rs = __builtin_amdgcn_make_buffer_rsrc(const_cast<float*>(in) + (t < ntiles ? t * 32 * d : 0), 0,
                                                          (int)(rows * rowb), 0x00020000);
#pragma unroll
        for (int r = 0; r < 32; ++r)
            pf[r] = __uint_as_float(__builtin_amdgcn_raw_buffer_load_b32(rs, voff, r * rowb, 0));
    }
    for (; t < ntiles; t += nwaves) {
        const int64_t base = t * 32;
        const int rows = (int)(B - base < 32 ? B - base : 32);
        const float* W = (WLDS ? lds : packed) + opaque_zero();
        float xmax = 0.f;
#pragma unroll
        for (int r = 0; r < 32; ++r) {
            xt[r * S + lane] = pf[r];
            xmax = tmax(xmax, fabsf(pf[r]));
        }
        if constexpr (SAMPLE) {
            const auto rs = __builtin_amdgcn_make_buffer_rsrc(made_draw_arg(draw...).z + base * d, 0, rows * rowb,
                                                              0x00020000);
#pragma unroll
            for (int r = 0; r < 32; ++r)
                __builtin_amdgcn_raw_buffer_store_b32(__float_as_uint(pf[r]), rs, voff, r * rowb, 0);
        }
        const bool dense = __builtin_amdgcn_ballot_w64(!(xmax <= tsafe)) != 0;
        wave_lds_sync();

        f32x16 h1[HT];
#pragma unroll
        for (int ht = 0; ht < HT; ++ht) {
            f32x16 a = load_bias16(W + L.b1 + ht * 32, h);
            const int nkc = dense ? L.NKC : nk1[ht];
            for (int kc = 0; kc < nkc; ++kc) {
#pragma unroll
                for (int g = 0; g < 4; ++g) {
                    const f32x4 w =
                        *reinterpret_cast<const f32x4*>(W + L.w1 + ((ht * 4 * L.NKC + kc * 4 + g) * 64 + lane) * 4);
#pragma unroll
                    for (int rr = 0; rr < 4; ++rr) a = mfma32(w[rr], xt[col * S + 32 * kc + 8 * g + 2 * rr + h], a);
                }
            }
#pragma unroll
            for (int r = 0; r < 16; ++r) a[r] = trelu(a[r]);
            h1[ht] = a;
        }
        f32x16 h2[HT];
        made_hidden_nk<HT>(W, L.w2, L.b2, h1, h2, nk2, dense || full2);
        made_hidden_nk<HT>(W, L.w3, L.b3, h2, h1, nk3, dense || full3);

        const float ldin = ldpf;
        if constexpr (SAMPLE) {
            made_draw_tile(pf, t + nwaves, ntiles, B, d, made_draw_arg(draw...).seed, draw_off);
        } else {
            const int64_t tn = t + nwaves;
            ldpf = (accumulate && tn < ntiles && lane < 32 && tn * 32 + col < B) ? logdet[tn * 32 + col] : 0.f;
            const int64_t rn = tn < ntiles ? (B - tn * 32 < 32 ? B - tn * 32 : 32) : 0;
            const auto rs = __builtin_amdgcn_make_buffer_rsrc(const_cast<float*>(in) + (tn < ntiles ? tn * 32 * d : 0), 0,
                                                              (int)(rn * rowb), 0x00020000);
#pragma unroll
            for (int r = 0; r < 32; ++r)
                pf[r] = __uint_as_float(__builtin_amdgcn_raw_buffer_load_b32(rs, voff, r * rowb, 0));
        }

        float acc = 0.f;
        for (int j = 0; j < L.NJ; ++j) {
            f32x16 mu, al;
            out_pair_n<HT, HT>(dense ? HT : nkp[L.nk4 + j], W, L, j, h1, mu, al);
#pragma unroll
            for (int r = 0; r < 16; ++r) {
                float* p = xt + col * S + 32 * j + crow(r, h);
                *p = made_affine<VAR>(*p, mu[r], al[r], acc);
            }
        }
        const float ssum = halves_sum(acc, acc);
        wave_lds_sync();
        float zsq = 0.f;
        if constexpr (LOGP) {
            if (lane < 32) {
                for (int jd = 0; jd < d; ++jd) {
                    const float v = xt[col * S + jd];
                    zsq = (jd == 0) ? gauss_sq0(v) : gauss_sq(zsq, v);
                }
            }
        }
        {
            const auto rs = __builtin_amdgcn_make_buffer_rsrc(out + base * d, 0, rows * rowb, 0x00020000);
#pragma unroll
            for (int r = 0; r < 32; ++r)
                __builtin_amdgcn_raw_buffer_store_b32(__float_as_uint(xt[r * S + lane]), rs, voff, r * rowb, 0);
        }
        if (lane < 32 && col < rows) {
            float ldv;
            if constexpr (VAR == NFX_MAF_INVERSE) {
                ldv = -ssum;
                if (nonfinite(ldv)) ldv = 0.f;
                ldv = tclamp(ldv, -100.f, 100.f);
            } else {
                ldv = ssum;
                if (nonfinite(ldv)) ldv = 0.f;
                ldv = tclamp(ldv, -50.f, 50.f);
            }
            const int64_t so = base + col;
            const float ldt = accumulate ? ldin + ldv : ldv;
            logdet[so] = ldt;
            if constexpr (LOGP) {
                const float lp = gauss_lp(zsq, cgauss, ldt);
                logp[so] = lp;
                lpacc += (double)lp;
            }
        }
        wave_lds_sync();
    }
    if constexpr (LOGP) {
        logp_commit<512>(lpacc, partials, sums, B);
    }
    if constexpr (SAMPLE) {
        rng_commit(made_draw_arg(draw...).rng);
    }
}

typedef void (*made_par_kernel_t)(const float*, const float*, float*, float*, int64_t, int, int, int64_t,
                                  float*, double*, double*, float);

template <int HT>
made_par_kernel_t made_pick_ht(bool wlds, int variant);
template <int HT>
made_par_kernel_t made_tile_pick_ht(bool wlds, int variant, bool logp);
template <int HT>
made_seq_kernel_t made_seq_pick_ht(int variant);
typedef void (*made_sample_kernel_t)(const float*, const float*, float*, float*, int64_t, int, int, int64_t, float*,
                                     double*, double*, float, MadeDraw);
template <int HT>
made_sample_kernel_t made_tile_sample_pick_ht(bool wlds);

}
```

### normalizing-flows-study_amd/csrc/nfx_made_sample.hip

```cpp
#include "nfx_made_kernel.h"

namespace nfx {

template <int HT>
made_sample_kernel_t made_tile_sample_pick_ht(bool wlds) {
    return wlds ? made_tile_kernel<HT, true, NFX_IAF_FORWARD, false, true, MadeDraw>
                : made_tile_kernel<HT, false, NFX_IAF_FORWARD, false, true, MadeDraw>;
}
template made_sample_kernel_t made_tile_sample_pick_ht<1>(bool);
template made_sample_kernel_t made_tile_sample_pick_ht<2>(bool);
template made_sample_kernel_t made_tile_sample_pick_ht<3>(bool);
template made_sample_kernel_t made_tile_sample_pick_ht<4>(bool);

}
```

### normalizing-flows-study_amd/nfs_amd/_lib.py

```python
import ctypes
import os
import threading
import types

import torch

_HERE = os.path.dirname(os.path.abspath(__file__))
LIB_PATH = os.environ.get("NFX_LIB", os.path.join(_HERE, "libnfx.so"))

NFX_OK = 0
NFX_EINVAL = -1
NFX_EUNSUPPORTED = -2
NFX_ELAUNCH = -3
NFX_FORWARD = 1
NFX_INVERSE = -1
NFX_MAF_INVERSE = 0
NFX_IAF_FORWARD = 1
NFX_MAF_FORWARD = 2
NFX_IAF_INVERSE = 3
NFX_AFFINE_AUTO = 0
NFX_AFFINE_STREAMING = 1
NFX_AFFINE_SMALL = 2
NFX_MADE_SEQ_AUTO = 0
NFX_MADE_SEQ_SEGMENT = 1
NFX_MADE_SEQ_WAVE = 2
NFX_MADE_SEQ_PUSH = 3
NFX_RESIDUAL_RELU = 0
NFX_RESIDUAL_ELU = 1
NFX_RESIDUAL_LEAKY_RELU = 2
NFX_RESIDUAL_TANH = 3
NFX_NAF_RELU = 0
NFX_NAF_ELU = 1
NFX_NAF_LEAKY_RELU = 2
NFX_NAF_GELU = 3
NFX_NAF_LAYER_NORM = 1


def NFX_NAF_RESIDUAL(l):
    return 2 << l


class NfxLibraryError(RuntimeError):
    pass


class NfxError(RuntimeError):
    pass


class NfxMlpRaw(ctypes.Structure):
    _fields_ = [
        ("w", ctypes.c_void_p * 4),
        ("b", ctypes.c_void_p * 4),
        ("mask", ctypes.c_void_p * 4),
        ("bn_w", ctypes.c_void_p * 3),
        ("bn_b", ctypes.c_void_p * 3),
        ("bn_rm", ctypes.c_void_p * 3),
        ("bn_rv", ctypes.c_void_p * 3),
        ("bn_eps", ctypes.c_float),
        ("n_layers", ctypes.c_int),
    ]


class NfxNafLayer(ctypes.Structure):
    _fields_ = [
        ("weight", ctypes.c_void_p),
        ("bias", ctypes.c_void_p),
        ("mask", ctypes.c_void_p),
        ("ln_weight", ctypes.c_void_p),
        ("ln_bias", ctypes.c_void_p),
        ("ln_eps", ctypes.c_float),
        ("residual", ctypes.c_int),
    ]


class NfxNafLayerGrad(ctypes.Structure):
    _fields_ = [
        ("weight", ctypes.c_void_p),
        ("bias", ctypes.c_void_p),
        ("ln_weight", ctypes.c_void_p),
        ("ln_bias", ctypes.c_void_p),
    ]


_vp = ctypes.c_void_p
_i64 = ctypes.c_int64
_int = ctypes.c_int
_f = ctypes.c_float
_sz = ctypes.c_size_t

_SIGNATURES = {
    "nfx_abi_version": (_int, []),
    "nfx_last_error": (ctypes.c_char_p, []),
    "nfx_last_kernel": (ctypes.c_char_p, []),
    "nfx_debug_fill_lds": (ctypes.c_int, [ctypes.c_uint32, ctypes.c_void_p]),
    "nfx_affine_packed_floats": (_sz, [_int, _int]),
    "nfx_affine_pack": (_int, [ctypes.POINTER(NfxMlpRaw), ctypes.POINTER(NfxMlpRaw), _vp, _int, _int, _vp, _vp]),
    "nfx_affine_coupling": (_int, [_vp, _vp, _vp, _vp, _i64, _int, _int, _int, _int, _vp]),
    "nfx_affine_coupling_logprob": (_int, [_vp, _vp, _vp, _vp, _vp, _vp, _vp, _i64, _int, _int, _int, _vp]),
    "nfx_affine_kernel_policy": (_int, [_int]),
    "nfx_linear_forward": (_int, [_vp, _vp, _vp, _vp, _vp, _vp, _vp, _vp, _i64, _int, _int, _int, _vp]),
    "nfx_linear_backward_data": (_int, [_vp, _vp, _vp, _vp, _vp, _vp, _i64, _int, _int, _int, _vp]),
    "nfx_linear_workspace_bytes": (_sz, [_i64, _int, _int]),
    "nfx_linear_backward_weight": (_int, [_vp, _vp, _vp, _vp, _vp, _vp, _i64, _int, _int, _vp, _vp]),
    "nfx_made_elem_forward": (_int, [_vp, _vp, _vp, _vp, _i64, _int, _int, _int, _vp]),
    "nfx_made_elem_step": (_int, [_vp, _vp, _vp, _vp, _i64, _int, _int, _int, _vp]),
    "nfx_made_elem_finish": (_int, [_vp, _vp, _vp, _vp, _vp, _i64, _int, _int, _int, _vp]),
    "nfx_made_elem_backward": (_int, [_vp, _vp, _vp, _vp, _vp, _vp, _i64, _int, _int, _vp]),
    "nfx_made_elem_seq_backward": (_int, [_vp, _vp, _vp, _vp, _vp, _vp, _vp, _i64, _int, _int, _int, _vp]),
    "nfx_made_elem_seq_step_backward": (_int, [_vp, _vp, _vp, _vp, _vp, _vp, _vp, _vp, _vp, _i64, _int, _int, _int,
                                               _vp]),
    "nfx_made_elem_prefix": (_int, [_vp, _vp, _i64, _int, _int, _vp]),
    "nfx_affine_elem_forward": (_int, [_vp, _vp, _vp, _vp, _vp, _vp, _i64, _int, _int, _int, _vp]),
    "nfx_affine_elem_backward": (_int, [_vp, _vp, _vp, _vp, _vp, _vp, _vp, _vp, _vp, _i64, _int, _int, _vp]),
    "nfx_bn_prepare": (_int, [_vp, _vp, _vp, _vp, _vp, ctypes.c_double, ctypes.c_double, _int, _int, _vp, _vp, _vp,
                              _vp, _vp]),
    "nfx_bn_apply_relu": (_int, [_vp, _vp, _vp, _vp, _i64, _int, _vp]),
    "nfx_arqs_step": (_int, [_vp, _vp, _vp, _vp, _vp, _vp, _vp, _vp, _i64, _int, _int, _int, _int, _int, _f, _f, _f,
                             _vp]),
    "nfx_bn_workspace_bytes": (_sz, [_i64, _int]),
    "nfx_bn_backward_sums": (_int, [_vp, _vp, _vp, _vp, _vp, _i64, _int, _vp, _vp]),
    "nfx_bn_backward_apply": (_int, [_vp, _vp, _vp, _vp, _vp, _vp, _vp, _int, _vp, _i64, _int, _vp]),
    "nfx_spline_elem_forward": (_int, [_vp, _vp, _vp, _vp, _vp, _i64, _int, _int, _f, _f, _f, _f, _int, _int, _vp]),
    "nfx_spline_elem_backward": (_int, [_vp, _vp, _vp, _vp, _vp, _vp, _vp, _i64, _int, _int, _f, _f, _f, _f, _int,
                                        _vp]),
    "nfx_spline_elem_forward_bounded": (_int, [_vp, _vp, _vp, _vp, _vp, _vp, _i64, _int, _int, _f, _f, _f, _f, _int,
                                               _int, _vp]),
    "nfx_spline_elem_backward_bounded": (_int, [_vp, _vp, _vp, _vp, _vp, _vp, _vp, _vp, _i64, _int, _int, _f, _f, _f,
                                                _f, _int, _vp]),
    "nfx_spline_rescale": (_int, [_vp, _vp, _vp, _i64, _int, _f, _vp]),
    "nfx_arqs_bounds": (_int, [_vp, _vp, _vp, _i64, _int, _int, _vp]),
    "nfx_affine_chain_supported": (_int, [_i64, _int, _int]),
    "nfx_affine_chain": (_int, [ctypes.POINTER(_vp), _int, _vp, _vp, _vp, _i64, _int, _int, _int, _int, _vp]),
    "nfx_affine_chain_logprob": (_int, [ctypes.POINTER(_vp), _int, _vp, _vp, _vp, _vp, _vp, _vp, _i64, _int, _int,
                                        _int, _vp]),
    "nfx_affine_chain_sample": (_int, [ctypes.POINTER(_vp), _int, ctypes.c_uint64, _vp, _vp, _vp, _vp, _i64, _int, _int,
                                       _vp]),
    "nfx_arqs_packed_floats": (_sz, [_int, _int, _int]),
    "nfx_arqs_pack": (_int, [ctypes.POINTER(NfxMlpRaw), _int, _int, _int, _vp, _vp]),
    "nfx_arqs": (_int, [_vp, _vp, _vp, _vp, _i64, _int, _int, _int, _f, _f, _f, _int, ctypes.c_double,
                        ctypes.c_double, _int, _int, _vp]),
    "nfx_spline_packed_floats": (_sz, [_int, _int, _int]),
    "nfx_spline_pack": (_int, [ctypes.POINTER(NfxMlpRaw), _vp, _int, _int, _int, _vp, _vp]),
    "nfx_spline_coupling": (_int, [_vp, _vp, _vp, _vp, _i64, _int, _int, _int, _f, _f, _f, _f,
                                   _int, _f, _f, _int, _int, _vp]),
    "nfx_spline_coupling_logprob": (_int, [_vp, _vp, _vp, _vp, _vp, _vp, _vp, _i64, _int, _int, _int, _f, _f,
                                           _f, _f, _int, _f, _f, _int, _vp]),
    "nfx_spline_chain_supported": (_int, [_i64, _int, _int, _int]),
    "nfx_spline_chain": (_int, [ctypes.POINTER(_vp), _int, _vp, _vp, _vp, _i64, _int, _int, _int, _f, _f, _f, _f,
                                _int, _int, _vp]),
    "nfx_spline_chain_logprob": (_int, [ctypes.POINTER(_vp), _int, _vp, _vp, _vp, _vp, _vp, _vp, _i64, _int, _int,
                                        _int, _f, _f, _f, _f, _int, _vp]),
    "nfx_spline_chain_sample": (_int, [ctypes.POINTER(_vp), _int, ctypes.c_uint64, _vp, _vp, _vp, _vp, _i64, _int, _int,
                                       _int, _f, _f, _f, _f, _vp]),
    "nfx_cnf_packed_floats": (_sz, [_int, _int]),
    "nfx_cnf_pack": (_int, [_vp, _vp, _vp, _vp, _vp, _vp, _int, _int, _vp, _vp]),
    "nfx_cnf_supported": (_int, [_i64, _int, _int]),
    "nfx_cnf_integrate": (_int, [_vp, _vp, _vp, _vp, _i64, _int, _int, _f, _f, _f, _int, _vp]),
    "nfx_cnf_backward_supported": (_int, [_i64, _int, _int]),
    "nfx_cnf_backward_packed_floats": (_sz, [_int, _int]),
    "nfx_cnf_trajectory_floats": (_sz, [_i64, _int, _f, _f, _f]),
    "nfx_cnf_backward_workspace_floats": (_sz, [_i64, _int, _int]),
    "nfx_cnf_backward_slots": (_sz, [_i64, _int, _int]),
    "nfx_cnf_backward_block_threads": (_sz, [_i64, _int, _int]),
    "nfx_cnf_pack_backward": (_int, [_vp, _vp, _vp, _vp, _vp, _vp, _int, _int, _vp, _vp]),
    "nfx_cnf_integrate_save": (_int, [_vp, _vp, _vp, _vp, _vp, _i64, _int, _int, _f, _f, _f, _int, _vp]),
    "nfx_cnf_backward": (_int, [_vp] * 16 + [_i64, _int, _int, _f, _f, _f, _vp]),
    "nfx_residual_packed_floats": (_sz, [_int, _int]),
    "nfx_residual_supported": (_int, [_i64, _int, _int, _int]),
    "nfx_residual_pack": (_int, [_vp, _vp, _vp, _vp, _f] * 3 + [_int, _int, _vp, _vp]),
    "nfx_residual_flow": (_int, [_vp, _vp, _vp, _vp, _i64, _int, _int, _int, _int, _int, _int, _f, _int, _vp]),
    "nfx_residual_backward_supported": (_int, [_i64, _int, _int, _int]),
    "nfx_residual_backward_packed_floats": (_sz, [_int, _int]),
    "nfx_residual_backward_workspace_floats": (_sz, [_i64, _int, _int]),
    "nfx_residual_backward_slots": (_sz, [_i64, _int, _int]),
    "nfx_residual_backward_block_threads": (_sz, [_i64, _int, _int]),
    "nfx_residual_pack_backward": (_int, [_vp, _vp, _vp, _vp, _f] * 3 + [_int, _int, _vp, _vp]),
    "nfx_residual_backward": (_int, [_vp] * 12 + [_i64, _int, _int, _int, _int, _int, _vp]),
    "nfx_naf_packed_floats": (_sz, [_int, _int, _vp]),
    "nfx_naf_supported": (_int, [_i64, _int, _int, _vp, _int, _int]),
    "nfx_naf_pack": (_int, [_vp, _int, _int, _vp, _vp, _vp]),
    "nfx_naf_flow": (_int, [_vp, _vp, _vp, _vp, _i64, _int, _int, _vp, _int, _int, _f, _f, _int, _int, _vp]),
    "nfx_naf_wide_packed_floats": (_sz, [_int, _int, _vp]),
    "nfx_naf_wide_supported": (_int, [_i64, _int, _int, _vp, _int, _int]),
    "nfx_naf_wide_pack": (_int, [_vp, _int, _int, _vp, _vp, _vp]),
    "nfx_naf_wide_flow": (_int, [_vp, _vp, _vp, _vp, _i64, _int, _int, _vp, _int, _int, _f, _f, _int, _int, _vp]),
    "nfx_naf_backward_supported": (_int, [_i64, _int, _int, _vp, _int, _int]),
    "nfx_naf_backward_packed_floats": (_sz, [_int, _int, _vp]),
    "nfx_naf_pack_backward": (_int, [_vp, _int, _int, _vp, _vp, _vp]),
    "nfx_naf_backward_slots": (_sz, [_i64, _int, _int, _vp]),
    "nfx_naf_backward_block_threads": (_sz, [_i64, _int, _int, _vp]),
    "nfx_naf_backward_workspace_floats": (_sz, [_i64, _int, _int, _vp]),
    "nfx_naf_backward": (_int, [_vp] * 8 + [_i64, _int, _int, _vp, _int, _int, _f, _f, _vp]),
    "nfx_lowrank_supported": (_int, [_i64, _int, _int]),
    "nfx_lowrank_record_floats": (_sz, [_int]),
    "nfx_lowrank_pack_planar": (_int, [_vp, _vp, _vp, _int, _int, _f, _vp, _vp]),
    "nfx_lowrank_pack_radial": (_int, [_vp, _vp, _vp, _int, _int, _f, _vp, _vp]),
    "nfx_lowrank_pack_sylvester": (_int, [_vp, _vp, _vp, _int, _int, _int, _int, _f, _vp, _vp]),
    "nfx_lowrank_stack": (_int, [_vp, _int, _vp, _vp, _vp, _i64, _int, _int, _int, _vp]),
    "nfx_lrbwd_supported": (_int, [_i64, _int, _int, _int]),
    "nfx_lrbwd_max_layers": (_sz, [_int]),
    "nfx_lrbwd_chunk_rows": (_sz, [_int]),
    "nfx_lrbwd_slots": (_sz, [_i64, _int, _int]),
    "nfx_lrbwd_workspace_floats": (_sz, [_i64, _int, _int]),
    "nfx_lrbwd_stack": (_int, [_vp, _int, _vp, _vp, _vp, _vp, _vp, _i64, _int, _int, _vp]),
    "nfx_lrbwd_param_grads": (_int, [_vp, _i64, _int, _int, _int, _int, _vp, _vp, _vp, _vp, _vp, _vp, _int, _int, _vp]),
    "nfx_rqs_unit": (_int, [_vp, _vp, _vp, _vp, _vp, _vp, _i64, _int, _f, _f, _f, _int, _vp]),
    "nfx_rqs_unit_backward": (_int, [_vp, _vp, _vp, _vp, _vp, _vp, _vp, _vp, _vp, _vp, _i64, _int, _f, _f, _f, _int,
                                     _vp]),
    "nfx_made_packed_floats": (_sz, [_int, _int]),
    "nfx_made_pack": (_int, [ctypes.POINTER(NfxMlpRaw), _int, _int, _vp, _vp]),
    "nfx_made_pack_parallel": (_int, [ctypes.POINTER(NfxMlpRaw), _int, _int, _vp, _vp]),
    "nfx_made_pack_sequential": (_int, [_int, _int, _vp, _vp]),
    "nfx_made_seq_policy": (_int, [_int]),
    "nfx_base_normal": (_int, [ctypes.c_uint64, _vp, _vp, _i64, _int, _vp]),
    "nfx_made_sample_supported": (_int, [_int, _int, _int]),
    "nfx_made_affine_sample": (_int, [_vp, ctypes.c_uint64, _vp, _vp, _vp, _vp, _i64, _int, _int, _vp]),
    "nfx_made_affine": (_int, [_vp, _vp, _vp, _vp, _i64, _int, _int, _int, _int, _vp]),
    "nfx_made_affine_logprob": (_int, [_vp, _vp, _vp, _vp, _vp, _vp, _vp, _i64, _int, _int, _int, _int, _vp]),
    "nfx_made_pack_backward": (_int, [ctypes.POINTER(NfxMlpRaw), _int, _int, _vp, _vp]),
    "nfx_made_backward_factor_floats": (_sz, [_i64, _int, _int]),
    "nfx_made_backward_max_batch": (_i64, [_int, _int]),
    "nfx_made_affine_backward": (_int, [_vp, _vp, _vp, _vp, _vp, _vp, _i64, _int, _int, _int, _vp]),
    "nfx_made_seq_backward": (_int, [_vp, _vp, _vp, _vp, _vp, _vp, _i64, _int, _int, _int, _vp]),
    "nfx_made_factor_pitch": (_i64, [_i64]),
    "nfx_made_param_floats": (_sz, [_int, _int]),
    "nfx_made_wgrad_workspace_bytes": (_sz, [_i64, _int, _int]),
    "nfx_made_backward_weights": (_int, [_vp, _i64, _int, _int, ctypes.POINTER(_vp), _vp, _vp, _vp]),
    "nfx_affine_train_pack_floats": (_sz, [_int, _int]),
    "nfx_affine_train_stats_doubles": (_sz, [_int]),
    "nfx_affine_train_grad_doubles": (_sz, [_int, _int]),
    "nfx_affine_train_param_floats": (_sz, [_int, _int]),
    "nfx_affine_train_workspace_bytes": (_sz, [_i64, _int, _int]),
    "nfx_affine_train_pack": (_int, [ctypes.POINTER(NfxMlpRaw), ctypes.POINTER(NfxMlpRaw), _vp, _vp, _vp, _int,
                                     _int, _vp, _vp, _vp]),
    "nfx_affine_train_stats": (_int, [_vp, _vp, _i64, _int, _int, _int, _vp, _vp, _vp]),
    "nfx_affine_train_update_running": (_int, [_vp, _vp, ctypes.POINTER(_vp), ctypes.POINTER(_vp), _int,
                                               ctypes.c_double, _vp]),
    "nfx_affine_train_update_running_counted": (_int, [_vp, _vp, ctypes.POINTER(_vp), ctypes.POINTER(_vp),
                                                       ctypes.POINTER(_vp), _int, ctypes.c_double, _vp]),
    "nfx_affine_train_backward": (_int, [_vp, _vp, _vp, _vp, _vp, _i64, _int, _int, _int, _int, _vp, _vp, _vp,
                                         _vp]),
    "nfx_affine_train_assemble": (_int, [_vp, _vp, _vp, _int, _int, _f, _vp, _vp]),
    "nfx_affine_train_keep_floats": (_sz, [_i64, _int, _int]),
    "nfx_affine_train_stats_keep": (_int, [_vp, _vp, _i64, _int, _int, _int, _vp, _vp, _vp, _vp]),
    "nfx_affine_train_backward_keep": (_int, [_vp, _vp, _vp, _vp, _vp, _i64, _int, _int, _int, _int, _vp, _vp,
                                              _vp, _vp, _vp]),
    "nfx_affine_train_output": (_int, [_vp, _vp, _vp, _vp, _vp, _i64, _int, _int, _int, _vp]),
    "nfx_affine_eval_stats": (_int, [ctypes.POINTER(_vp), ctypes.POINTER(_vp), _int, _vp, _vp, _vp]),
    "nfx_spline_backward_packed_floats": (_sz, [_int, _int, _int]),
    "nfx_spline_backward_param_floats": (_sz, [_int, _int, _int]),
    "nfx_spline_backward_workspace_bytes": (_sz, [_i64, _int, _int, _int]),
    "nfx_spline_pack_backward": (_int, [ctypes.POINTER(NfxMlpRaw), _vp, _int, _int, _int, _vp, _vp]),
    "nfx_spline_coupling_backward": (_int, [_vp, _vp, _vp, _vp, _vp, _vp, _vp, _vp, _i64, _int, _int, _int, _int,
                                            _f, _f, _f, _f, _int, _vp]),
    "nfx_gauss_workspace_bytes": (_sz, [_i64]),
    "nfx_gauss_workspace_init": (_int, [_vp, _vp]),
    "nfx_gauss_logprob": (_int, [_vp, _vp, _vp, _vp, _vp, _i64, _int, _vp]),
    "nfx_gauss_logprob_backward": (_int, [_vp, _vp, _vp, _vp, _i64, _int, _vp]),
    "nfx_flowbn_workspace_bytes": (_sz, [_i64, _int]),
    "nfx_flowbn_apply": (_int, [_vp, _vp, _vp, _vp, _vp, _vp, _vp, _f, _i64, _int, _int, _vp]),
    "nfx_flowbn_moments": (_int, [_vp, _i64, _int, _vp, _vp, _vp]),
    "nfx_flowbn_update_running": (_int, [_vp, _vp, _vp, ctypes.c_double, _int, _vp]),
    "nfx_flowbn_backward": (_int, [_vp, _vp, _vp, _vp, _vp, _vp, _vp, _vp, _f, _vp, _vp, _i64, _int, _int,
                                   _vp, _vp]),
}

EXPORTED_SYMBOLS = tuple(_SIGNATURES)

_VALUE_RETURNING = frozenset((
    "nfx_abi_version", "nfx_affine_kernel_policy", "nfx_made_seq_policy", "nfx_affine_chain_supported",
    "nfx_spline_chain_supported", "nfx_cnf_supported", "nfx_cnf_backward_supported",
    "nfx_made_sample_supported", "nfx_residual_supported", "nfx_residual_backward_supported",
    "nfx_naf_supported", "nfx_naf_wide_supported", "nfx_naf_backward_supported",
    "nfx_lowrank_supported", "nfx_lrbwd_supported"))


_as_pointer = _vp.from_param


class DevicePtr:

    @staticmethod
    def from_param(v):
        if v is None or type(v) is int:
            return _as_pointer(v)
        return _as_pointer(v.data_ptr())


def _raise_on_status(rc, fn, args):
    if rc != NFX_OK:
        raise NfxError(f"{fn.__name__} failed (rc={rc}): {lib().nfx_last_error().decode(errors='replace')}")
    return rc


_lock = threading.Lock()
_lib = None
_checked = None


def load(path=LIB_PATH):
    global _lib, _checked
    with _lock:
        if _lib is not None:
            return _lib
        if not os.path.exists(path):
            raise NfxLibraryError(
                f"libnfx.so not found at {path}: build it with "
                f"`python normalizing-flows-study_amd/build.py` (or __graft_entry__.build()). "
                f"The HIP path has no eager fallback.")
        l = ctypes.CDLL(path)
        n = types.SimpleNamespace()
        for name, (res, args) in _SIGNATURES.items():
            fn = getattr(l, name, None)
            if fn is None:
                continue
            fn.restype = res
            fn.argtypes = args
            cf = l._FuncPtr((name, l))
            cf.__name__ = name
            cf.restype = res
            cf.argtypes = [DevicePtr if a is _vp else a for a in args]
            if res is _int and name not in _VALUE_RETURNING:
                cf.errcheck = _raise_on_status
            setattr(n, name, cf)
        _checked = n
        _lib = l
        return l


def lib():
    l = _lib
    return l if l is not None else load()


def checked():
    if _checked is None:
        load()
    return _checked


def available():
    try:
        load()
        return True
    except NfxLibraryError:
        return False


def check(rc, what):
    if rc != NFX_OK:
        msg = lib().nfx_last_error().decode(errors="replace")
        raise NfxError(f"{what} failed (rc={rc}): {msg}")


def dense(t):
    t = t.contiguous()
    if t.data_ptr() & 15:
        t = t.clone()
    return t


def ptr(t):
    return None if t is None else t.data_ptr()


try:
    _raw_stream = torch._C._cuda_getCurrentRawStream
except AttributeError:
    _raw_stream = None


def stream_of(t):
    if _raw_stream is not None and t.device.type == "cuda":
        return _raw_stream(t.device.index if t.device.index is not None else torch.cuda.current_device())
    return torch.cuda.current_stream(t.device).cuda_stream


def mlp_raw(linears, batchnorms=(), masks=None):
    raw = NfxMlpRaw()
    keep = []

    def p(t):
        t = dense(t.detach().float())
        keep.append(t)
        return t.data_ptr()

    raw.n_layers = len(linears)
    for i, lin in enumerate(linears):
        raw.w[i] = p(lin.weight)
        raw.b[i] = p(lin.bias) if lin.bias is not None else None
        if masks is not None and masks[i] is not None:
            raw.mask[i] = p(masks[i])
    eps = 1e-5
    for i, bn in enumerate(batchnorms):
        if bn is None:
            continue
        raw.bn_w[i] = p(bn.weight) if bn.weight is not None else p(torch.ones_like(bn.running_var))
        raw.bn_b[i] = p(bn.bias) if bn.bias is not None else p(torch.zeros_like(bn.running_var))
        raw.bn_rm[i] = p(bn.running_mean)
        raw.bn_rv[i] = p(bn.running_var)
        eps = bn.eps
    raw.bn_eps = eps
    return raw, keep


def last_kernel():
    return lib().nfx_last_kernel().decode()
```

Measured before the change: 1.614 billion.

## Add split-bf16 MFMA tile path for MADE hidden and output layers

Measured after the change: 1.613 billion. About the same (-0.0%).

```diff
diff --git a/include/nfx.h b/include/nfx.h
--- a/include/nfx.h
+++ b/include/nfx.h
@@ -119,6 +119,11 @@
 #define NFX_MADE_SEQ_WAVE 2
 #define NFX_MADE_SEQ_PUSH 3
 int nfx_made_seq_policy(int policy);
+#define NFX_MADE_TILE_AUTO 0
+#define NFX_MADE_TILE_FP32 1
+#define NFX_MADE_TILE_SPLIT 2
+int nfx_made_tile_policy(int policy);
+size_t nfx_made_split_offset(int d, int H);
 int nfx_made_affine_logprob(const float* packed, const float* in, float* out, float* log_det,
                             float* logp, double* sums, void* workspace, int64_t B, int d, int H,
                             int variant, int accumulate, void* stream);
diff --git a/normalizing-flows-study_amd/csrc/nfx_affine_kernel.h b/normalizing-flows-study_amd/csrc/nfx_affine_kernel.h
--- a/normalizing-flows-study_amd/csrc/nfx_affine_kernel.h
+++ b/normalizing-flows-study_amd/csrc/nfx_affine_kernel.h
@@ -3,6 +3,7 @@
 #include <utility>
 
 #include "nfx_common.h"
+#include "nfx_split.h"
 
 namespace nfx {
 
@@ -150,39 +151,6 @@
         res[j] = tclamp(halves_sum(part[j][0], part[j][1]) + P[L.b3 + j], -10.f, 10.f);
 }
 
-#ifndef NFX_SPLIT_TERMS
-#define NFX_SPLIT_TERMS 6
-#endif
-typedef __bf16 bf16x8 __attribute__((ext_vector_type(8)));
-typedef uint32_t u32x4 __attribute__((ext_vector_type(4)));
-
-__device__ __forceinline__ f32x16 mfma_bf16(u32x4 a, u32x4 b, f32x16 c) {
-    return __builtin_amdgcn_mfma_f32_32x32x16_bf16(__builtin_bit_cast(bf16x8, a), __builtin_bit_cast(bf16x8, b), c,
-                                                    0, 0, 0);
-}
-
-__device__ __forceinline__ void split3(float x, uint32_t& u0, uint32_t& u1, uint32_t& u2) {
-    u0 = __float_as_uint(x) & 0xffff0000u;
-    const float r1 = x - __uint_as_float(u0);
-    u1 = __float_as_uint(r1) & 0xffff0000u;
-    u2 = __float_as_uint(r1 - __uint_as_float(u1));
-}
-
-__device__ __forceinline__ uint32_t pack_bf16(uint32_t lo, uint32_t hi) {
-    return __builtin_amdgcn_perm(hi, lo, 0x07060302u);
-}
-
-__device__ __forceinline__ void split_block(const f32x16& a, int half, u32x4 (&xp)[3]) {
-#pragma unroll
-    for (int q = 0; q < 4; ++q) {
-        uint32_t l0, l1, l2, h0, h1, h2;
-        split3(a[8 * half + 2 * q], l0, l1, l2);
-        split3(a[8 * half + 2 * q + 1], h0, h1, h2);
-        xp[0][q] = pack_bf16(l0, h0);
-        xp[1][q] = pack_bf16(l1, h1);
-        xp[2][q] = pack_bf16(l2, h2);
-    }
-}
 
 template <class F, int... I>
 __device__ __forceinline__ void static_for_seq(F&& f, std::integer_sequence<int, I...>) {
@@ -193,11 +161,6 @@
     static_for_seq(f, std::make_integer_sequence<int, N>{});
 }
 
-#if NFX_SPLIT_TERMS == 8
-constexpr int kSplitTermW[8] = {2, 1, 2, 1, 0, 1, 0, 0}, kSplitTermX[8] = {1, 2, 0, 1, 2, 0, 1, 0};
-#else
-constexpr int kSplitTermW[6] = {2, 1, 0, 1, 0, 0}, kSplitTermX[6] = {0, 1, 2, 0, 1, 0};
-#endif
 
 template <int HT, int D, int TILES, bool LIVE>
 __device__ __forceinline__ void affine_nets_split_pipe(const float* __restrict__ S, const AffineSplit& SL,
diff --git a/normalizing-flows-study_amd/csrc/nfx_made.hip b/normalizing-flows-study_amd/csrc/nfx_made.hip
--- a/normalizing-flows-study_amd/csrc/nfx_made.hip
+++ b/normalizing-flows-study_amd/csrc/nfx_made.hip
@@ -135,6 +135,97 @@
     }
 }
 
+__global__ __launch_bounds__(kLiveThreads) void made_split_pack_kernel(NfxMlpRaw net, MadeSplit S, int d, int H,
+                                                                       float* packed) {
+    const int HT = (H + 31) / 32;
+    const MadeLayout L = made_layout(d, HT);
+    const int Hp = L.Hp;
+    float* out = packed + L.split + kMadeSplitHdr;
+    const int sb2 = L.w2, sb3 = sb2 + HT * 32, sb4 = sb3 + HT * 32, sblk = sb4 + L.NJ * 64;
+    __shared__ int bad;
+    __shared__ unsigned rmax[3];
+    __shared__ double red[2 * kLiveThreads / 64];
+    if (threadIdx.x < 3) rmax[threadIdx.x] = 0u;
+    if (threadIdx.x == 0) bad = 0;
+    __syncthreads();
+    bool b = false;
+    for (int i = threadIdx.x; i < S.img; i += kLiveThreads) {
+        uint32_t v;
+        if (i < sb2) {
+            v = __float_as_uint(packed[L.w1 + i]);
+        } else if (i < sb3) {
+            v = __float_as_uint(packed[L.b2 + (i - sb2)]);
+        } else if (i < sb4) {
+            v = __float_as_uint(packed[L.b3 + (i - sb3)]);
+        } else if (i < sblk) {
+            v = __float_as_uint(packed[L.b4 + (i - sb4)]);
+        } else {
+            const int t = (i - sblk) % kMadeSplitBlock, blk = (i - sblk) / kMadeSplitBlock;
+            const int q = t & 3, lane = (t >> 2) & 63, p = (t >> 8) % 3, kbl = (t >> 8) / 3;
+            int woff = 0, tile = 0;
+            for (int hto = 0; hto < HT; ++hto) {
+                if (blk >= S.blk2[hto] && blk < S.blk2[hto] + S.ext2[hto]) woff = L.w2, tile = a_tile(hto, blk - S.blk2[hto], HT);
+                if (blk >= S.blk3[hto] && blk < S.blk3[hto] + S.ext3[hto]) woff = L.w3, tile = a_tile(hto, blk - S.blk3[hto], HT);
+            }
+            for (int j = 0; j < L.NJ; ++j)
+                if (blk >= S.blk4[j] && blk < S.blk4[j] + 2 * S.ext4[j]) {
+                    const int w = (blk - S.blk4[j]) / S.ext4[j], kt = (blk - S.blk4[j]) % S.ext4[j];
+                    woff = L.w4, tile = a_tile(2 * j + w, kt, HT);
+                }
+            uint32_t half[2];
+            for (int e = 0; e < 2; ++e) {
+                const int r = 8 * kbl + 2 * q + e;
+                const float w = packed[woff + (a_quad(tile, r >> 2) * 64 + lane) * 4 + (r & 3)];
+                const uint32_t u0 = __builtin_bit_cast(uint16_t, (__bf16)w);
+                const float r1 = w - __uint_as_float(u0 << 16);
+                const uint32_t u1 = __builtin_bit_cast(uint16_t, (__bf16)r1);
+                const uint32_t u2 = __builtin_bit_cast(uint16_t, (__bf16)(r1 - __uint_as_float(u1 << 16)));
+                half[e] = p == 0 ? u0 : p == 1 ? u1 : u2;
+            }
+            v = half[0] | (half[1] << 16);
+        }
+        out[i] = __uint_as_float(v);
+    }
+    for (int i = threadIdx.x; i < 2 * Hp + 2 * d; i += kLiveThreads) {
+        const int layer = i < Hp ? 0 : i < 2 * Hp ? 1 : 2;
+        const float* row = packed + (layer == 0 ? L.s_w2 + i * Hp : layer == 1 ? L.s_w3 + (i - Hp) * Hp
+                                                                                : L.s_w4 + (i - 2 * Hp) * Hp);
+        float sum = 0.f;
+        for (int k = 0; k < Hp; ++k) {
+            const float a = fabsf(row[k]);
+            if (!(a <= 1e6f)) b = true;
+            sum += a;
+        }
+        if (sum <= 3e38f) atomicMax(&rmax[layer], __float_as_uint(sum));
+        else b = true;
+    }
+    const int* nk = reinterpret_cast<const int*>(packed);
+    if (threadIdx.x < HT && (nk[L.nk2 + threadIdx.x] > S.ext2[threadIdx.x] || nk[L.nk3 + threadIdx.x] > S.ext3[threadIdx.x]))
+        b = true;
+    if (threadIdx.x < L.NJ && nk[L.nk4 + threadIdx.x] > S.ext4[threadIdx.x]) b = true;
+    if (b) atomicOr(&bad, 1);
+    const int rows[4] = {H, H, H, 2 * d}, cols[4] = {d, H, H, H};
+    const double xs30 = block_mlp_tsafe(net, 4, rows, cols, 1.0e30, red);
+    if (threadIdx.x == 0) {
+        const double r2 = __uint_as_float(rmax[0]), r3 = __uint_as_float(rmax[1]), r4 = __uint_as_float(rmax[2]);
+        const bool lost = !(0x1p-133 * (r2 * r3 * r4 + r3 * r4 + r4) < 0x1p-100);
+        const float xs = (float)fmin(xs30, (double)packed[L.tsafe]);
+        int* hdr = reinterpret_cast<int*>(packed + L.split);
+        hdr[0] = (!bad && !lost && xs > 0.f) ? 1 : 0;
+        packed[L.split + 1] = xs > 0.f ? xs : 0.f;
+        for (int i = 0; i < 2; ++i) {
+            hdr[2 + i] = S.ext2[i];
+            hdr[4 + i] = S.ext3[i];
+            hdr[6 + i] = S.ext4[i];
+            hdr[8 + i] = S.blk2[i];
+            hdr[10 + i] = S.blk3[i];
+            hdr[12 + i] = S.blk4[i];
+        }
+        hdr[14] = S.img;
+        hdr[15] = 0;
+    }
+}
+
 template <int HT>
 made_seqs_kernel_t made_seqs_pick_ht(int variant, bool logp) {
     if (variant == NFX_MAF_FORWARD) return made_seqs_kernel<HT, NFX_MAF_FORWARD, false>;
@@ -223,7 +314,10 @@
         const int groups = HT * 4 * L.NKC + 2 * HT * HT * 4 + L.NJ * 2 * HT * 4;
         made_extent_kernel<<<(groups + 3) / 4, 256, 0, (hipStream_t)stream>>>(d, H, packed);
     }
-    return check_launch("made_extent_kernel");
+    rc = check_launch("made_extent_kernel");
+    if (rc || !made_has_split(d, (H + 31) / 32)) return rc;
+    made_split_pack_kernel<<<1, kLiveThreads, 0, (hipStream_t)stream>>>(*net, made_split(d, H), d, H, packed);
+    return check_launch("made_split_pack_kernel");
 }
 
 extern "C" int nfx_made_pack_sequential(int d, int H, float* packed, void* stream) {
@@ -260,6 +354,23 @@
 int made_seq_policy_get() { return made_seq_policy().load(std::memory_order_relaxed); }
 }
 
+static std::atomic<int>& made_tile_policy() {
+    static std::atomic<int> v{[] {
+        const char* e = getenv("NFX_MADE_TILE_POLICY");
+        const int p = e ? atoi(e) : NFX_MADE_TILE_AUTO;
+        return p >= NFX_MADE_TILE_AUTO && p <= NFX_MADE_TILE_SPLIT ? p : NFX_MADE_TILE_AUTO;
+    }()};
+    return v;
+}
+
+static bool tile_split_auto(int d, int H) { return H > 32 && d > 32; }
+
+static bool tile_split(int d, int H) {
+    if (!made_has_split(d, (H + 31) / 32) || d > 64) return false;
+    const int pol = made_tile_policy().load(std::memory_order_relaxed);
+    return pol == NFX_MADE_TILE_SPLIT || (pol == NFX_MADE_TILE_AUTO && tile_split_auto(d, H));
+}
+
 static bool tile_path(int d, int HT, int variant) {
     return (variant == NFX_MAF_INVERSE || variant == NFX_IAF_FORWARD) && d > 0 && d <= kTileMaxD && HT >= 1 && HT <= 4;
 }
@@ -269,10 +380,10 @@
     bool wlds;
     size_t lds;
 };
-static TileConfig tile_config(const MadeLayout& L, int64_t ntiles, bool fused) {
+static TileConfig tile_config(const MadeLayout& L, int64_t ntiles, bool fused, int split_img = 0) {
     int nw = 8;
     if (!fused && ntiles < 4 * (int64_t)num_cus()) nw = (int)((ntiles + num_cus() - 1) / num_cus());
-    const size_t wbytes = (size_t)L.par_total * sizeof(float);
+    const size_t wbytes = (size_t)(split_img ? split_img : L.par_total) * sizeof(float);
     const size_t tiles = nw * 32 * (size_t)kTileStride * sizeof(float);
     const bool wlds = nw == 8 && wbytes + tiles <= kLdsBytes;
     return {nw, wlds, (wlds ? wbytes : 0) + tiles};
@@ -323,8 +434,11 @@
     }
     if (tile_path(d, HT, variant)) {
         const int64_t ntiles = (B + 31) / 32;
-        const TileConfig c = tile_config(L, ntiles, fused);
-        made_par_kernel_t k = pick_tile(HT, c.wlds, variant, fused);
+        const bool split = tile_split(d, H);
+        const TileConfig c = tile_config(L, ntiles, fused, split ? made_split(d, H).img : 0);
+        made_par_kernel_t k = !split    ? pick_tile(HT, c.wlds, variant, fused)
+                              : HT == 1 ? made_tile_split_pick_ht<1>(c.wlds, variant, fused)
+                                        : made_tile_split_pick_ht<2>(c.wlds, variant, fused);
         if (!k) return set_error(NFX_EUNSUPPORTED, "made_affine: no kernel for H=%d", H);
         int rc = prepare_lds((const void*)k, c.lds);
         if (rc) return rc;
@@ -388,6 +502,17 @@
     return made_seq_policy().exchange(policy);
 }
 
+extern "C" int nfx_made_tile_policy(int policy) {
+    if (policy < 0) return made_tile_policy().load();
+    if (policy > NFX_MADE_TILE_SPLIT) return set_error(NFX_EINVAL, "made_tile_policy: unknown policy %d", policy);
+    return made_tile_policy().exchange(policy);
+}
+
+extern "C" size_t nfx_made_split_offset(int d, int H) {
+    if (d <= 0 || H <= 0 || !made_has_split(d, (H + 31) / 32)) return 0;
+    return (size_t)made_layout(d, (H + 31) / 32).split;
+}
+
 extern "C" int nfx_made_affine(const float* packed, const float* in, float* out, float* log_det,
                                int64_t B, int d, int H, int variant, int accumulate, void* stream) {
     return made_launch(packed, in, out, log_det, B, d, H, variant, accumulate, nullptr, nullptr, nullptr,
@@ -418,9 +543,12 @@
     const int HT = (H + 31) / 32;
     const MadeLayout L = made_layout(d, HT);
     const int64_t ntiles = (B + 31) / 32;
-    const TileConfig c = tile_config(L, ntiles, false);
+    const bool split = tile_split(d, H);
+    const TileConfig c = tile_config(L, ntiles, false, split ? made_split(d, H).img : 0);
     made_sample_kernel_t k =
-        pick_range<1, 4>(HT, [=](auto HT_) { return made_tile_sample_pick_ht<HT_()>(c.wlds); });
+        !split    ? pick_range<1, 4>(HT, [=](auto HT_) { return made_tile_sample_pick_ht<HT_()>(c.wlds); })
+        : HT == 1 ? made_tile_split_sample_pick_ht<1>(c.wlds)
+                  : made_tile_split_sample_pick_ht<2>(c.wlds);
     int rc = prepare_lds((const void*)k, c.lds);
     if (rc) return rc;
     int grid = resident_grid((const void*)k, 64 * c.nw, c.lds, (ntiles + c.nw - 1) / c.nw);
diff --git a/normalizing-flows-study_amd/csrc/nfx_made_kernel.h b/normalizing-flows-study_amd/csrc/nfx_made_kernel.h
--- a/normalizing-flows-study_amd/csrc/nfx_made_kernel.h
+++ b/normalizing-flows-study_amd/csrc/nfx_made_kernel.h
@@ -1,6 +1,7 @@
 #pragma once
 #include "nfx_common.h"
 #include "nfx_rng.h"
+#include "nfx_split.h"
 
 namespace nfx {
 
@@ -15,8 +16,23 @@
     int sw1, sw4, sb4;
     int ctab;
     int ps, pw4, pw1, pb4, pw23, ptb, ptab;
+    int split;
     int total;
 };
+
+constexpr int kMadeSplitHdr = 16;
+constexpr int kMadeSplitBlock = 2 * 3 * 64 * 4;
+struct MadeSplit {
+    int ext2[2], ext3[2], ext4[2], blk2[2], blk3[2], blk4[2];
+    int nblk, img;
+};
+__host__ __device__ constexpr bool made_has_split(int d, int HT) { return d <= 64 && HT <= 2; }
+__host__ __device__ constexpr int made_split_max_floats(int d, int HT) {
+    const int NJ = (d + 31) / 32;
+    return made_has_split(d, HT) ? kMadeSplitHdr + HT * 4 * NJ * 256 + 4 * HT * 32 + NJ * 64 +
+                                       (2 * HT * HT + NJ * 2 * HT) * kMadeSplitBlock
+                                 : 0;
+}
 
 __host__ __device__ constexpr int made_up4(int v) { return (v + 3) & ~3; }
 
@@ -80,8 +96,46 @@
     L.pw23 = o; o += PS ? 2 * L.Hp * L.Hp : 0;
     L.ptb = o; o += PS ? 4 * L.Hp : 0;
     L.ptab = o; o += PS ? 16 * seqp_max_chunks(d, L.Hp) : 0;
+    o = made_up4(o);
+    L.split = o; o += made_split_max_floats(d, HT);
     L.total = o;
     return L;
+}
+
+inline int made_ref_degree(int a, int d, int H) {
+    if (d <= 1 || H <= 1) return 0;
+    if (d == 2) return (a >> 1) & 1;
+    if (a == H - 1) return d - 1;
+    return (int)((double)a * ((double)(d - 1) / (double)(H - 1)));
+}
+
+inline MadeSplit made_split(int d, int H) {
+    const int HT = (H + 31) / 32, NJ = (d + 31) / 32;
+    const MadeLayout L = made_layout(d, HT);
+    MadeSplit S{};
+    int n = 0;
+    for (int layer = 0; layer < 2; ++layer)
+        for (int hto = 0; hto < HT; ++hto) {
+            int ext = 0;
+            for (int a = 32 * hto; a < 32 * hto + 32 && a < H; ++a)
+                for (int b = 0; b < H; ++b)
+                    if (made_ref_degree(b, d, H) <= made_ref_degree(a, d, H) && b / 32 + 1 > ext) ext = b / 32 + 1;
+            (layer ? S.ext3 : S.ext2)[hto] = ext;
+            (layer ? S.blk3 : S.blk2)[hto] = n;
+            n += ext;
+        }
+    for (int j = 0; j < NJ; ++j) {
+        int ext = 0;
+        for (int i = 32 * j; i < 32 * j + 32 && i < d; ++i)
+            for (int b = 0; b < H; ++b)
+                if (made_ref_degree(b, d, H) < i && b / 32 + 1 > ext) ext = b / 32 + 1;
+        S.ext4[j] = ext;
+        S.blk4[j] = n;
+        n += 2 * ext;
+    }
+    S.nblk = n;
+    S.img = L.w2 + 2 * HT * 32 + NJ * 64 + n * kMadeSplitBlock;
+    return S;
 }
 
 constexpr int kStageStride = 33;
@@ -507,6 +561,87 @@
     }
 }
 
+template <int HT>
+__device__ __forceinline__ void split_acts(const f32x16 (&hin)[HT], u32x4 (&xp)[2 * HT][3]) {
+#pragma unroll
+    for (int kb = 0; kb < 2 * HT; ++kb) split_block(hin[kb >> 1], kb & 1, xp[kb]);
+}
+
+__device__ __forceinline__ void split_kblock(const float* __restrict__ Wb, int kb, const u32x4 (&xp)[3],
+                                             f32x16& hi, f32x16& lo) {
+    const u32x4* wp = reinterpret_cast<const u32x4*>(Wb) + kb * 3 * 64 + lane_id();
+    const u32x4 w[3] = {wp[0], wp[64], wp[128]};
+#pragma unroll
+    for (int t = 0; t < NFX_SPLIT_TERMS; ++t) {
+        if (t < NFX_SPLIT_TERMS - 1) lo = mfma_bf16(w[kSplitTermW[t]], xp[kSplitTermX[t]], lo);
+        else hi = mfma_bf16(w[kSplitTermW[t]], xp[kSplitTermX[t]], hi);
+    }
+}
+
+__device__ __forceinline__ f32x16 zero16() {
+    f32x16 z;
+#pragma unroll
+    for (int r = 0; r < 16; ++r) z[r] = 0.f;
+    return z;
+}
+
+template <int HT, int NK>
+__device__ __forceinline__ f32x16 hidden_tile_split(const float* __restrict__ Wb, const float* __restrict__ bias,
+                                                    const u32x4 (&xp)[2 * HT][3]) {
+    f32x16 hi = load_bias16(bias, lane_id() >> 5), lo = zero16();
+#pragma unroll
+    for (int kb = 0; kb < 2 * NK; ++kb) split_kblock(Wb, kb, xp[kb], hi, lo);
+#pragma unroll
+    for (int r = 0; r < 16; ++r) hi[r] = trelu(hi[r] + lo[r]);
+    return hi;
+}
+
+template <int HT, int N>
+__device__ __forceinline__ f32x16 hidden_tile_split_n(int n, const float* __restrict__ Wb,
+                                                      const float* __restrict__ bias, const u32x4 (&xp)[2 * HT][3]) {
+    if constexpr (N == 0) {
+        return hidden_tile_split<HT, 0>(Wb, bias, xp);
+    } else {
+        if (n >= N) return hidden_tile_split<HT, N>(Wb, bias, xp);
+        return hidden_tile_split_n<HT, N - 1>(n, Wb, bias, xp);
+    }
+}
+
+template <int HT, int NK>
+__device__ __forceinline__ void out_pair_split(const float* __restrict__ Wm, const float* __restrict__ Wa,
+                                               const float* __restrict__ bias, const u32x4 (&xp)[2 * HT][3],
+                                               f32x16& mu, f32x16& al) {
+    const int h = lane_id() >> 5;
+    mu = load_bias16(bias, h);
+    al = load_bias16(bias + 32, h);
+    f32x16 mlo = zero16(), alo = zero16();
+#pragma unroll
+    for (int kb = 0; kb < 2 * NK; ++kb) {
+        split_kblock(Wm, kb, xp[kb], mu, mlo);
+        split_kblock(Wa, kb, xp[kb], al, alo);
+    }
+#pragma unroll
+    for (int r = 0; r < 16; ++r) {
+        mu[r] = mu[r] + mlo[r];
+        al[r] = al[r] + alo[r];
+    }
+}
+
+template <int HT, int N>
+__device__ __forceinline__ void out_pair_split_n(int n, const float* __restrict__ Wm, const float* __restrict__ Wa,
+                                                 const float* __restrict__ bias, const u32x4 (&xp)[2 * HT][3],
+                                                 f32x16& mu, f32x16& al) {
+    if constexpr (N == 0) {
+        out_pair_split<HT, 0>(Wm, Wa, bias, xp, mu, al);
+    } else {
+        if (n >= N) {
+            out_pair_split<HT, N>(Wm, Wa, bias, xp, mu, al);
+            return;
+        }
+        out_pair_split_n<HT, N - 1>(n, Wm, Wa, bias, xp, mu, al);
+    }
+}
+
 struct MadeDraw {
     uint64_t seed;
     uint64_t* rng;
@@ -528,7 +663,31 @@
     }
 }
 
-template <int HT, bool WLDS, int VAR, bool LOGP, bool SAMPLE = false, typename... DRAW>
+template <int HT>
+__device__ __forceinline__ void tile_layer1(const float* __restrict__ W, const MadeLayout& L, const float* xt,
+                                            bool dense, const int (&nk1)[HT], f32x16 (&h1)[HT]) {
+    constexpr int S = kTileStride;
+    const int lane = lane_id(), h = lane >> 5, col = lane & 31;
+#pragma unroll
+    for (int ht = 0; ht < HT; ++ht) {
+        f32x16 a = load_bias16(W + L.b1 + ht * 32, h);
+        const int nkc = dense ? L.NKC : nk1[ht];
+        for (int kc = 0; kc < nkc; ++kc) {
+#pragma unroll
+            for (int g = 0; g < 4; ++g) {
+                const f32x4 w =
+                    *reinterpret_cast<const f32x4*>(W + L.w1 + ((ht * 4 * L.NKC + kc * 4 + g) * 64 + lane) * 4);
+#pragma unroll
+                for (int rr = 0; rr < 4; ++rr) a = mfma32(w[rr], xt[col * S + 32 * kc + 8 * g + 2 * rr + h], a);
+            }
+        }
+#pragma unroll
+        for (int r = 0; r < 16; ++r) a[r] = trelu(a[r]);
+        h1[ht] = a;
+    }
+}
+
+template <int HT, bool WLDS, int VAR, bool LOGP, bool SPLIT = false, bool SAMPLE = false, typename... DRAW>
 __global__ __launch_bounds__(512) void made_tile_kernel(
     const float* __restrict__ packed, const float* __restrict__ in, float* __restrict__ out,
     float* __restrict__ logdet, int64_t B, int d, int accumulate, int64_t ntiles,
@@ -536,23 +695,26 @@
     DRAW... draw) {
     static_assert(sizeof...(DRAW) == (SAMPLE ? 1 : 0), "SAMPLE kernels take one MadeDraw");
     static_assert(!SAMPLE || (VAR == NFX_IAF_FORWARD && !LOGP), "SAMPLE: the IAF forward pass");
+    static_assert(!SPLIT || HT <= 2, "SPLIT: H <= 64");
     const MadeLayout L = made_layout(d, HT);
+    const int* nkp = reinterpret_cast<const int*>(packed);
+    const int wimg = SPLIT ? nkp[L.split + 14] : L.par_total;
+    const float* wsrc = packed + (SPLIT ? L.split + kMadeSplitHdr : 0);
     constexpr int S = kTileStride;
     extern __shared__ f32x4 lds4[];
     float* lds = reinterpret_cast<float*>(lds4);
     const int wave = __builtin_amdgcn_readfirstlane(threadIdx.x >> 6);
     const int nwg = LOGP ? 8 : (int)(blockDim.x >> 6);
     if constexpr (WLDS) {
-        const f32x4* src = reinterpret_cast<const f32x4*>(packed);
-        for (int i = threadIdx.x; i < L.par_total / 4; i += 64 * nwg) lds4[i] = src[i];
-    }
-    float* xt = lds + (WLDS ? L.par_total : 0) + wave * 32 * S;
+        const f32x4* src = reinterpret_cast<const f32x4*>(wsrc);
+        for (int i = threadIdx.x; i < wimg / 4; i += 64 * nwg) lds4[i] = src[i];
+    }
+    float* xt = lds + (WLDS ? wimg : 0) + wave * 32 * S;
     if constexpr (WLDS) __syncthreads();
     const int lane = lane_id(), h = lane >> 5, col = lane & 31;
     const int64_t nwaves = (int64_t)gridDim.x * nwg;
     const int voff = lane < d ? lane * 4 : (1 << 30);
     const int rowb = d * 4;
-    const int* nkp = reinterpret_cast<const int*>(packed);
     int nk1[HT], nk2[HT], nk3[HT];
     bool full2 = true, full3 = true;
 #pragma unroll
@@ -564,6 +726,18 @@
         full3 = full3 && nk3[i] >= HT;
     }
     const float tsafe = packed[L.tsafe];
+    const int* hp = nkp + L.split;
+    const bool ok = SPLIT && hp[0] != 0;
+    const float xs = SPLIT ? packed[L.split + 1] : 0.f;
+    int e2[HT], e3[HT], o2[HT], o3[HT];
+#pragma unroll
+    for (int i = 0; i < HT; ++i) {
+        e2[i] = SPLIT ? hp[2 + i] : 0;
+        e3[i] = SPLIT ? hp[4 + i] : 0;
+        o2[i] = SPLIT ? hp[8 + i] * kMadeSplitBlock : 0;
+        o3[i] = SPLIT ? hp[10 + i] * kMadeSplitBlock : 0;
+    }
+    const int sb2 = L.w2, sb3 = sb2 + HT * 32, sb4 = sb3 + HT * 32, sblk = sb4 + L.NJ * 64;
 
     int64_t t = (int64_t)blockIdx.x * nwg + wave;
     double lpacc = 0.0;
@@ -585,7 +759,7 @@
     for (; t < ntiles; t += nwaves) {
         const int64_t base = t * 32;
         const int rows = (int)(B - base < 32 ? B - base : 32);
-        const float* W = (WLDS ? lds : packed) + opaque_zero();
+        const float* W = (WLDS ? lds : wsrc) + opaque_zero();
         float xmax = 0.f;
 #pragma unroll
         for (int r = 0; r < 32; ++r) {
@@ -603,26 +777,45 @@
         wave_lds_sync();
 
         f32x16 h1[HT];
-#pragma unroll
-        for (int ht = 0; ht < HT; ++ht) {
-            f32x16 a = load_bias16(W + L.b1 + ht * 32, h);
-            const int nkc = dense ? L.NKC : nk1[ht];
-            for (int kc = 0; kc < nkc; ++kc) {
-#pragma unroll
-                for (int g = 0; g < 4; ++g) {
-                    const f32x4 w =
-                        *reinterpret_cast<const f32x4*>(W + L.w1 + ((ht * 4 * L.NKC + kc * 4 + g) * 64 + lane) * 4);
-#pragma unroll
-                    for (int rr = 0; rr < 4; ++rr) a = mfma32(w[rr], xt[col * S + 32 * kc + 8 * g + 2 * rr + h], a);
-                }
-            }
-#pragma unroll
-            for (int r = 0; r < 16; ++r) a[r] = trelu(a[r]);
-            h1[ht] = a;
-        }
-        f32x16 h2[HT];
-        made_hidden_nk<HT>(W, L.w2, L.b2, h1, h2, nk2, dense || full2);
-        made_hidden_nk<HT>(W, L.w3, L.b3, h2, h1, nk3, dense || full3);
+        f32x16 hf[HT];
+        u32x4 xp[SPLIT ? 2 * HT : 1][3];
+        bool runf = false, uns = false, densef = dense;
+        if constexpr (!SPLIT) {
+            tile_layer1<HT>(W, L, xt, dense, nk1, h1);
+            f32x16 h2[HT];
+            made_hidden_nk<HT>(W, L.w2, L.b2, h1, h2, nk2, dense || full2);
+            made_hidden_nk<HT>(W, L.w3, L.b3, h2, h1, nk3, dense || full3);
+        } else {
+            const float* G = packed + opaque_zero();
+            runf = uns = !ok;
+            if (ok && __builtin_amdgcn_ballot_w64(!(xmax <= xs)) != 0) {
+                float m = 0.f;
+                for (int k = 0; k < d; ++k) m = tmax(m, fabsf(xt[col * S + k]));
+                uns = !(m <= xs);
+                runf = densef = true;
+            }
+#pragma unroll
+            for (int i = 0; i < HT; ++i) hf[i] = zero16();
+            if (runf) {
+                f32x16 ha[HT], hb[HT];
+                tile_layer1<HT>(G, L, xt, densef, nk1, ha);
+                made_hidden_nk<HT>(G, L.w2, L.b2, ha, hb, nk2, densef || full2);
+                made_hidden_nk<HT>(G, L.w3, L.b3, hb, hf, nk3, densef || full3);
+            }
+            if (ok) {
+                tile_layer1<HT>(W, L, xt, false, nk1, h1);
+                f32x16 h2[HT];
+                split_acts<HT>(h1, xp);
+#pragma unroll
+                for (int i = 0; i < HT; ++i)
+                    h2[i] = hidden_tile_split_n<HT, HT>(e2[i], W + sblk + o2[i], W + sb2 + i * 32, xp);
+                split_acts<HT>(h2, xp);
+#pragma unroll
+                for (int i = 0; i < HT; ++i)
+                    h1[i] = hidden_tile_split_n<HT, HT>(e3[i], W + sblk + o3[i], W + sb3 + i * 32, xp);
+                split_acts<HT>(h1, xp);
+            }
+        }
 
         const float ldin = ldpf;
         if constexpr (SAMPLE) {
@@ -641,7 +834,26 @@
         float acc = 0.f;
         for (int j = 0; j < L.NJ; ++j) {
             f32x16 mu, al;
-            out_pair_n<HT, HT>(dense ? HT : nkp[L.nk4 + j], W, L, j, h1, mu, al);
+            if constexpr (!SPLIT) {
+                out_pair_n<HT, HT>(dense ? HT : nkp[L.nk4 + j], W, L, j, h1, mu, al);
+            } else {
+                if (ok) {
+                    const int e4 = hp[6 + j];
+                    const float* Wm = W + sblk + hp[12 + j] * kMadeSplitBlock;
+                    out_pair_split_n<HT, HT>(e4, Wm, Wm + e4 * kMadeSplitBlock, W + sb4 + j * 64, xp, mu, al);
+                } else {
+                    mu = al = zero16();
+                }
+                if (runf) {
+                    f32x16 muf, alf;
+                    out_pair_n<HT, HT>(densef ? HT : nkp[L.nk4 + j], packed + opaque_zero(), L, j, hf, muf, alf);
+#pragma unroll
+                    for (int r = 0; r < 16; ++r) {
+                        mu[r] = uns ? muf[r] : mu[r];
+                        al[r] = uns ? alf[r] : al[r];
+                    }
+                }
+            }
 #pragma unroll
             for (int r = 0; r < 16; ++r) {
                 float* p = xt + col * S + 32 * j + crow(r, h);
@@ -708,5 +920,9 @@
                                      double*, double*, float, MadeDraw);
 template <int HT>
 made_sample_kernel_t made_tile_sample_pick_ht(bool wlds);
-
-}
+template <int HT>
+made_par_kernel_t made_tile_split_pick_ht(bool wlds, int variant, bool logp);
+template <int HT>
+made_sample_kernel_t made_tile_split_sample_pick_ht(bool wlds);
+
+}
diff --git a/normalizing-flows-study_amd/csrc/nfx_made_sample.hip b/normalizing-flows-study_amd/csrc/nfx_made_sample.hip
--- a/normalizing-flows-study_amd/csrc/nfx_made_sample.hip
+++ b/normalizing-flows-study_amd/csrc/nfx_made_sample.hip
@@ -4,8 +4,8 @@
 
 template <int HT>
 made_sample_kernel_t made_tile_sample_pick_ht(bool wlds) {
-    return wlds ? made_tile_kernel<HT, true, NFX_IAF_FORWARD, false, true, MadeDraw>
-                : made_tile_kernel<HT, false, NFX_IAF_FORWARD, false, true, MadeDraw>;
+    return wlds ? made_tile_kernel<HT, true, NFX_IAF_FORWARD, false, false, true, MadeDraw>
+                : made_tile_kernel<HT, false, NFX_IAF_FORWARD, false, false, true, MadeDraw>;
 }
 template made_sample_kernel_t made_tile_sample_pick_ht<1>(bool);
 template made_sample_kernel_t made_tile_sample_pick_ht<2>(bool);
diff --git a/normalizing-flows-study_amd/csrc/nfx_made_split.hip b/normalizing-flows-study_amd/csrc/nfx_made_split.hip
--- /dev/null
+++ b/normalizing-flows-study_amd/csrc/nfx_made_split.hip
@@ -0,0 +1,27 @@
+#include "nfx_made_kernel.h"
+
+namespace nfx {
+
+template <int HT, bool WLDS>
+static made_par_kernel_t tile_split_var(int variant, bool logp) {
+    if (variant != NFX_MAF_INVERSE) return made_tile_kernel<HT, WLDS, NFX_IAF_FORWARD, false, true>;
+    return logp ? made_tile_kernel<HT, WLDS, NFX_MAF_INVERSE, true, true>
+                : made_tile_kernel<HT, WLDS, NFX_MAF_INVERSE, false, true>;
+}
+
+template <int HT>
+made_par_kernel_t made_tile_split_pick_ht(bool wlds, int variant, bool logp) {
+    return wlds ? tile_split_var<HT, true>(variant, logp) : tile_split_var<HT, false>(variant, logp);
+}
+template made_par_kernel_t made_tile_split_pick_ht<1>(bool, int, bool);
+template made_par_kernel_t made_tile_split_pick_ht<2>(bool, int, bool);
+
+template <int HT>
+made_sample_kernel_t made_tile_split_sample_pick_ht(bool wlds) {
+    return wlds ? made_tile_kernel<HT, true, NFX_IAF_FORWARD, false, true, true, MadeDraw>
+                : made_tile_kernel<HT, false, NFX_IAF_FORWARD, false, true, true, MadeDraw>;
+}
+template made_sample_kernel_t made_tile_split_sample_pick_ht<1>(bool);
+template made_sample_kernel_t made_tile_split_sample_pick_ht<2>(bool);
+
+}
diff --git a/normalizing-flows-study_amd/csrc/nfx_split.h b/normalizing-flows-study_amd/csrc/nfx_split.h
--- /dev/null
+++ b/normalizing-flows-study_amd/csrc/nfx_split.h
@@ -0,0 +1,46 @@
+#pragma once
+#include "nfx_common.h"
+
+namespace nfx {
+
+#ifndef NFX_SPLIT_TERMS
+#define NFX_SPLIT_TERMS 6
+#endif
+typedef __bf16 bf16x8 __attribute__((ext_vector_type(8)));
+typedef uint32_t u32x4 __attribute__((ext_vector_type(4)));
+
+__device__ __forceinline__ f32x16 mfma_bf16(u32x4 a, u32x4 b, f32x16 c) {
+    return __builtin_amdgcn_mfma_f32_32x32x16_bf16(__builtin_bit_cast(bf16x8, a), __builtin_bit_cast(bf16x8, b), c,
+                                                    0, 0, 0);
+}
+
+__device__ __forceinline__ void split3(float x, uint32_t& u0, uint32_t& u1, uint32_t& u2) {
+    u0 = __float_as_uint(x) & 0xffff0000u;
+    const float r1 = x - __uint_as_float(u0);
+    u1 = __float_as_uint(r1) & 0xffff0000u;
+    u2 = __float_as_uint(r1 - __uint_as_float(u1));
+}
+
+__device__ __forceinline__ uint32_t pack_bf16(uint32_t lo, uint32_t hi) {
+    return __builtin_amdgcn_perm(hi, lo, 0x07060302u);
+}
+
+__device__ __forceinline__ void split_block(const f32x16& a, int half, u32x4 (&xp)[3]) {
+#pragma unroll
+    for (int q = 0; q < 4; ++q) {
+        uint32_t l0, l1, l2, h0, h1, h2;
+        split3(a[8 * half + 2 * q], l0, l1, l2);
+        split3(a[8 * half + 2 * q + 1], h0, h1, h2);
+        xp[0][q] = pack_bf16(l0, h0);
+        xp[1][q] = pack_bf16(l1, h1);
+        xp[2][q] = pack_bf16(l2, h2);
+    }
+}
+
+#if NFX_SPLIT_TERMS == 8
+constexpr int kSplitTermW[8] = {2, 1, 2, 1, 0, 1, 0, 0}, kSplitTermX[8] = {1, 2, 0, 1, 2, 0, 1, 0};
+#else
+constexpr int kSplitTermW[6] = {2, 1, 0, 1, 0, 0}, kSplitTermX[6] = {0, 1, 2, 0, 1, 0};
+#endif
+
+}
diff --git a/normalizing-flows-study_amd/nfs_amd/_lib.py b/normalizing-flows-study_amd/nfs_amd/_lib.py
--- a/normalizing-flows-study_amd/nfs_amd/_lib.py
+++ b/normalizing-flows-study_amd/nfs_amd/_lib.py
@@ -25,6 +25,9 @@
 NFX_MADE_SEQ_SEGMENT = 1
 NFX_MADE_SEQ_WAVE = 2
 NFX_MADE_SEQ_PUSH = 3
+NFX_MADE_TILE_AUTO = 0
+NFX_MADE_TILE_FP32 = 1
+NFX_MADE_TILE_SPLIT = 2
 NFX_RESIDUAL_RELU = 0
 NFX_RESIDUAL_ELU = 1
 NFX_RESIDUAL_LEAKY_RELU = 2
@@ -213,6 +216,8 @@
     "nfx_made_pack_parallel": (_int, [ctypes.POINTER(NfxMlpRaw), _int, _int, _vp, _vp]),
     "nfx_made_pack_sequential": (_int, [_int, _int, _vp, _vp]),
     "nfx_made_seq_policy": (_int, [_int]),
+    "nfx_made_tile_policy": (_int, [_int]),
+    "nfx_made_split_offset": (_sz, [_int, _int]),
     "nfx_base_normal": (_int, [ctypes.c_uint64, _vp, _vp, _i64, _int, _vp]),
     "nfx_made_sample_supported": (_int, [_int, _int, _int]),
     "nfx_made_affine_sample": (_int, [_vp, ctypes.c_uint64, _vp, _vp, _vp, _vp, _i64, _int, _int, _vp]),
@@ -269,7 +274,8 @@
 EXPORTED_SYMBOLS = tuple(_SIGNATURES)
 
 _VALUE_RETURNING = frozenset((
-    "nfx_abi_version", "nfx_affine_kernel_policy", "nfx_made_seq_policy", "nfx_affine_chain_supported",
+    "nfx_abi_version", "nfx_affine_kernel_policy", "nfx_made_seq_policy", "nfx_made_tile_policy",
+    "nfx_affine_chain_supported",
     "nfx_spline_chain_supported", "nfx_cnf_supported", "nfx_cnf_backward_supported",
     "nfx_made_sample_supported", "nfx_residual_supported", "nfx_residual_backward_supported",
     "nfx_naf_supported", "nfx_naf_wide_supported", "nfx_naf_backward_supported",
```
